# emmyoh/zebra

Hardware: AMD Instinct MI355X
Metric: queries/sec (higher is better)
Workload: dtype f32

## Files before the change

### zebra_amd/csrc/zh_api.hip

```cpp
#include <algorithm>
#include <atomic>
#include <chrono>
#include <condition_variable>
#include <cmath>
#include <deque>
#include <cstdarg>
#include <cstdio>
#include <cstring>
#include <mutex>
#include <shared_mutex>
#include <new>
#include <string>
#include <thread>
#include <vector>

#include "zh_internal.h"
#include "zh_snapfile.h"

static thread_local std::string g_err;

static int fail(int code, const char *fmt, ...) {
    char buf[512];
    va_list ap;
    va_start(ap, fmt);
    vsnprintf(buf, sizeof buf, fmt, ap);
    va_end(ap);
    g_err = buf;
    return code;
}
#define HIPCHK(expr)                                                                                       \
    do {                                                                                                   \
        hipError_t e_ = (expr);                                                                            \
        if (e_ != hipSuccess)                                                                              \
            return fail(e_ == hipErrorOutOfMemory ? ZH_ENOMEM : ZH_EHIP, "%s: %s (%s:%d)", #expr,          \
                        hipGetErrorString(e_), __FILE__, __LINE__);                                        \
    } while (0)

int zh_set_error(int code, const char *fmt, ...) {
    char buf[512];
    va_list ap;
    va_start(ap, fmt);
    vsnprintf(buf, sizeof buf, fmt, ap);
    va_end(ap);
    g_err = buf;
    return code;
}

extern "C" const char *zh_last_error(void) { return g_err.c_str(); }
extern "C" const char *zh_version(void) { return "zebra-hip 0.1 (gfx950)"; }

struct DevBuf {
    void *p = nullptr;
    size_t cap = 0;
    bool defer = false;
    std::vector<void *> old;
    size_t old_bytes = 0;
    int ensure(size_t bytes, bool keep = false, hipStream_t s = nullptr) {
        if (bytes <= cap) return ZH_OK;
        if (defer) bytes += bytes / 8;
        if (defer && old_bytes + cap > (size_t(2) << 30)) {
            for (void *o : old) hipFree(o);
            old.clear();
            old_bytes = 0;
        }
        size_t ncap = std::max(bytes, cap + cap / 2);
        ncap = (ncap + 255) & ~size_t(255);
        void *np = nullptr;
        hipError_t e = hipMalloc(&np, ncap);
        if (e != hipSuccess) {
            ncap = (bytes + 255) & ~size_t(255);
            e = hipMalloc(&np, ncap);
        }
        if (e != hipSuccess) return fail(ZH_ENOMEM, "hipMalloc(%zu bytes): %s", ncap, hipGetErrorString(e));
        if (keep && p && cap) {
            e = hipMemcpyAsync(np, p, cap, hipMemcpyDeviceToDevice, s);
            if (e == hipSuccess) e = hipStreamSynchronize(s);
            if (e != hipSuccess) { hipFree(np); return fail(ZH_EHIP, "grow copy: %s", hipGetErrorString(e)); }
        }
        if (p) { if (defer) { old.push_back(p); old_bytes += cap; } else hipFree(p); }
        p = np;
        cap = ncap;
        return ZH_OK;
    }
    void release() {
        if (p) hipFree(p);
        for (void *o : old) hipFree(o);
        old.clear();
        old_bytes = 0;
        p = nullptr;
        cap = 0;
    }
    template <typename T>
    T *as() const { return reinterpret_cast<T *>(p); }
};

struct zh_search_ctx {
    zh_index *ix = nullptr;
    DevBuf wQQ, wBits, wCounts, wInline, wRowBase, wCandBase, wVisitBase, wTotals, wVisits, wKeys, wCandKeys, wCandIds,
        wLeafCount, wLeafFill, wGroupBase, wGroupRowBase, wGroups, wGroupRowOff, wWaveGroup, wVisitBits, wNodeVisit, wScore, wJunkBits, wZeros, wQnorm, wQpad, wFixList, wLogPool, wLogHead, wLogCtl,
        wPfRows, wPfCounts, wPfKeys, wPfIds, wPfAmb, wPfCtl, wUnc, wQh, wQmeta, wApList, wApCount, wApEx, wApExKeys, wApCtl, wRaw;
    ZhApprox dbg_ap{};
    bool dbg_valid = false, dbg_raw = false;
    size_t log_chunks = 0;
    ZhTotals *h_totals = nullptr;
    hipEvent_t ev[6] = {};
    hipEvent_t ev_totals = nullptr, ev_emit = nullptr, ev_sw0 = nullptr, ev_sw1 = nullptr;
    bool ev_ok = false;
    int state = 0;
    bool trivial = false;
    const float *dQ = nullptr;
    size_t B = 0, k = 0;
    size_t nwin = 1, bwin = 0;
    DevBuf wQwin, wOutWin;
    int metric = 0, mode = 0;
    uint32_t P_dense = 0, wpq = 0;
    hipStream_t s = nullptr;
    ZhTotals tot{};
    bool scan = false;
    bool approx_f32rows = false;
    bool approx_fused = false;
    bool approx_bytes = false;
    bool approx = false, approx_mfma = false, approx_leaf = false;
    uint32_t *h_ap = nullptr;
    bool score_hash = false;
    uint32_t score_Bp = 0;
    bool lazy_fix = false;
    bool prefilter = false, prefilter_off_once = false, stream_ordered = false;
    uint32_t pf_cap = 0;
    uint32_t *h_pf = nullptr;
    std::vector<const float *> sv_q;
    std::vector<uint64_t *> sv_ids, sv_keys;
    std::vector<uint32_t *> sv_counts;
    hipStream_t sv_heavy = nullptr;
    std::vector<DevBuf *> all_bufs() {
        return {&wQQ, &wBits, &wCounts, &wInline, &wRowBase, &wCandBase, &wVisitBase, &wTotals, &wVisits, &wKeys,
                &wCandKeys, &wCandIds, &wLeafCount, &wLeafFill, &wGroupBase, &wGroupRowBase, &wGroups, &wGroupRowOff, &wWaveGroup, &wVisitBits, &wNodeVisit, &wScore, &wJunkBits, &wZeros, &wQnorm, &wQpad, &wFixList,
                &wLogPool, &wLogHead, &wLogCtl, &wQwin, &wOutWin, &wPfRows, &wPfCounts, &wPfKeys, &wPfIds, &wPfAmb, &wPfCtl, &wUnc,
                &wQh, &wQmeta, &wApList, &wApCount, &wApEx, &wApExKeys, &wApCtl, &wRaw};
    }
    void release_all() {
        for (DevBuf *b : all_bufs()) b->release();
        if (ev_ok) { for (auto &e : ev) hipEventDestroy(e); hipEventDestroy(ev_totals); hipEventDestroy(ev_emit); hipEventDestroy(ev_sw0); hipEventDestroy(ev_sw1); ev_ok = false; }
        if (h_totals) { hipHostFree(h_totals); h_totals = nullptr; }
        if (h_pf) { hipHostFree(h_pf); h_pf = nullptr; }
        if (h_ap) { hipHostFree(h_ap); h_ap = nullptr; }
    }
};

struct zh_index {
    zh_options opt{};
    int device = 0;
    hipStream_t stream = nullptr;
    hipStream_t sweep_stream = nullptr;
    std::shared_mutex mu;

    DevBuf X;
    uint64_t n_rows = 0;

    DevBuf node_plane, node_left, node_right, node_pack, roots, planes, consts, leaf_ids;
    uint32_t n_nodes = 0, n_planes = 0, n_trees = 0;
    uint64_t n_leaf_ids = 0;
    std::vector<int32_t> h_plane, h_left, h_right;
    std::vector<uint32_t> h_roots;
    std::vector<uint32_t> planes_below_level;
    std::vector<uint32_t> h_leaf_ids;
    std::vector<uint8_t> h_dead;
    uint64_t n_dead = 0;
    std::vector<uint32_t> h_live;
    uint64_t h_live_rows = ~0ull;
    uint64_t h_live_dead = ~0ull;
    uint64_t h_live_gen = ~0ull;
    uint64_t rows_gen = 1, dead_gen = 1;
    uint32_t max_leaf_len = 0;
    DevBuf blk_recs, blk_upper, blk_roots;
    uint32_t n_blocks = 0, n_upper = 0;
    bool blocks_valid = false;
    bool blocks_inner = false;
    size_t blk_recs_b = 0;
    std::mutex blk_mu;
    DevBuf row_leaf;
    bool row_leaf_valid = false, row_leaf_failed = false;
    std::atomic<uint32_t> batches_since_change{0};
    DevBuf row_half, row_meta, row_rho_dev;
    std::atomic<bool> row_half_failed{false};
    DevBuf row_half128;
    std::atomic<uint64_t> h128_rows{0}, h128_gen{0};
    int h128_ex = 0;
    float h128_rho = 0.f;
    std::atomic<bool> h128_failed{false};
    bool h128_bytes = false, h128_not_bytes = false;
    std::atomic<uint64_t> scale_rows{0}, scale_gen{0};
    float row_rho = 0.f;
    DevBuf scan_perm, row_leaf_p;
    bool row_order_off = false;
    uint32_t order_keys = 0;
    double order_worth = 0;
    uint64_t perm_rows = 0, row_leaf_gen = 0, row_leaf_p_gen = 0, perm_gen = 0, row_leaf_p_perm = 0;
    uint64_t row_leaf_rows = 0;

    zh_search_ctx dctx;
    DevBuf wQ, wOutIds, wOutKeys, wOutCounts;
    DevBuf ex_live, ex_bits, ex_QQ, ex_keys, ex_visits, ex_cbase, ex_ckeys, ex_cids, ex_run_ids, ex_run_keys, ex_run_counts, ex_Q, ex_ids, ex_kout, ex_counts,
        ex_Qh, ex_qmeta, ex_tau, ex_cnt, ex_lid, ex_llo, ex_lhi, ex_scr, ex_over;
    uint64_t ex_live_rows = ~0ull, ex_live_gen = ~0ull, ex_n_live = 0;
    zh_exact_info ex_info{};
    DevBuf fl_filter, fl_bits, fl_pos, fl_bcount, fl_bexcl, fl_tmp, fl_list;
    zh_filtered_info fl_info{};
    DevBuf rg_maxk, rg_cnt, rg_ctr, rg_pv0, rg_pv1, rg_pk0, rg_pk1, rg_cand, rg_tmp, rg_off, rg_oids, rg_okeys;
    zh_range_info rg_info{};
    DevBuf jn_ctr, jn_maxk, jn_tau, jn_pv0, jn_pv1, jn_pk0, jn_pk1, jn_qm, jn_cid, jn_first, jn_cand, jn_rows, jn_tmp, jn_oa, jn_ob, jn_okeys;
    zh_join_info jn_info{};
    DevBuf kn_qm, kn_cid, kn_pos, kn_A, kn_pmeta, kn_pid, kn_cbase, kn_pids, kn_pkeys, kn_pcounts, kn_oids, kn_okeys, kn_ocounts;
    zh_knn_info kn_info{};
    DevBuf fk_ntree, fk_rl, fk_flag, fk_excl, fk_tmp, fk_rows, fk_ctr, fk_lens, fk_takes, fk_rbase, fk_cbase, fk_groups, fk_groff, fk_segs, fk_colsrc, fk_crow,
        fk_hrow, fk_held, fk_CA, fk_cmeta, fk_cqm, fk_HA, fk_hmeta, fk_qrow, fk_maxk, fk_redo, fk_pos;
    zh_knn_forest_info fk_info{};
    DevBuf fj_leafof, fj_pieces, fj_linel, fj_linek, fj_segs, fj_cand;
    zh_join_forest_info fj_info{};

// ... 2082 lines not shown
    if (c->state != 1) return fail(ZH_ESTATE, "zh_search_finish without zh_search_begin");
    const uint32_t d = ix->opt.dim, T = ix->n_trees;
    const size_t B = c->B, k = c->k, nwin = c->nwin, bwin = c->bwin;
    hipStream_t s = c->s;
    int rc;
    c->state = 0;
    if (c->trivial) {
        for (size_t j = 0; j < nwin && bwin; j++) {
            HIPCHK(hipMemsetAsync(outCounts[j], 0, bwin * 4, s));
            if (k) {
                HIPCHK(hipMemsetAsync(outIds[j], 0xFF, bwin * k * 8, s));
                HIPCHK(hipMemsetAsync(outKeys[j], 0xFF, bwin * k * 8, s));
            }
        }
        HIPCHK(hipEventRecord(c->ev[5], s));
        c->state = 2;
        return ZH_OK;
    }
    uint64_t *dOutIds = outIds[0], *dOutKeys = outKeys[0];
    uint32_t *dOutCounts = outCounts[0];
    if (nwin > 1) {
        if ((rc = c->wOutWin.ensure(B * k * 16 + B * 4))) { return rc; }
        dOutIds = c->wOutWin.as<uint64_t>();
        dOutKeys = dOutIds + B * k;
        dOutCounts = reinterpret_cast<uint32_t *>(dOutKeys + B * k);
    }
    HIPCHK(hipEventSynchronize(c->ev_totals));
    const ZhTotals tot = c->tot = *c->h_totals;
    {
        std::lock_guard<std::mutex> lk(ix->stats_mu);
        const double v = (double)tot.visits / (double)((uint64_t)B * T);
        ix->visits_per_pair = ix->visits_per_pair > 0 ? 0.5 * (ix->visits_per_pair + v) : v;
    }
    if (tot.visits > 0xFFFFFFFull || tot.rows >= (1ull << 36))
        return fail(ZH_ELIMIT, "more than 2^28 leaf visits or 2^36 scored rows in one batch; use a smaller batch");
    c->sv_ids.assign(outIds, outIds + nwin); c->sv_keys.assign(outKeys, outKeys + nwin); c->sv_counts.assign(outCounts, outCounts + nwin);
    c->sv_heavy = heavy;
    if (c->prefilter && (tot.flags & 1u)) {
        const std::vector<const float *> q = c->sv_q;
        c->prefilter_off_once = true;
        rc = ctx_begin(c, q.data(), nwin, bwin, k, c->metric, c->mode, s);
        c->prefilter_off_once = false;
        if (rc) return rc;
        return ctx_finish(c, outIds, outKeys, outCounts, heavy);
    }
    if (c->prefilter) return finish_prefilter(c, dOutIds, dOutKeys, dOutCounts, outIds, outKeys, outCounts);
    if ((rc = c->wVisits.ensure(std::max<uint64_t>(tot.visits, 1) * sizeof(ZhVisit)))) return rc;
    if ((rc = c->wGroups.ensure(std::max<uint64_t>(tot.groups, 1) * sizeof(ZhGroup)))) return rc;
    if ((rc = c->wGroupRowOff.ensure(std::max<uint64_t>(tot.groups, 1) * 8))) return rc;
    if ((rc = c->wWaveGroup.ensure((tot.group_rows / 64 + 2) * 4))) return rc;
    if ((rc = c->wKeys.ensure(std::max<uint64_t>(tot.rows, 1) * 8))) return rc;
    if ((rc = c->wCandKeys.ensure(std::max<uint64_t>(tot.takes, 1) * 8))) return rc;
    if ((rc = c->wCandIds.ensure(std::max<uint64_t>(tot.takes, 1) * 4))) return rc;
    ZhForestDev f = forest_dev(ix);
    if (!(tot.flags & 1u)) {
        HIPCHK(zh_launch_expand(f, (uint32_t)B, c->wCounts.as<ZhPairCounts>(), c->wInline.as<ZhVisit>(),
                                c->wRowBase.as<uint64_t>(), c->wCandBase.as<uint64_t>(), c->wVisitBase.as<uint64_t>(),
                                c->wVisits.as<ZhVisit>(), c->wLeafCount.as<uint32_t>(), c->wLeafFill.as<uint32_t>(),
                                c->wGroupBase.as<uint32_t>(), c->wGroupRowBase.as<uint64_t>(), c->wGroups.as<ZhGroup>(),
                                c->wGroupRowOff.as<uint64_t>(), walk_log(c), s));
    } else {
        if (c->lazy_fix)
            HIPCHK(zh_launch_score_unc_fix(c->dQ, (uint32_t)B, d, f.planes, f.consts, ix->n_planes, c->wBits.as<uint32_t>(), c->wUnc.as<uint32_t>(), c->wpq, s));
        HIPCHK(zh_launch_walk_emit(f, c->dQ, (uint32_t)B, d, (int32_t)k, c->wBits.as<uint32_t>(), c->wpq, c->P_dense,
                                   c->wCounts.as<ZhPairCounts>(), c->wInline.as<ZhVisit>(), c->wRowBase.as<uint64_t>(),
                                   c->wCandBase.as<uint64_t>(), c->wVisitBase.as<uint64_t>(), c->wVisits.as<ZhVisit>(),
                                   c->wLeafCount.as<uint32_t>(), c->wLeafFill.as<uint32_t>(), c->wGroupBase.as<uint32_t>(),
                                   c->wGroupRowBase.as<uint64_t>(), c->wGroups.as<ZhGroup>(), c->wGroupRowOff.as<uint64_t>(), s));
        const uint64_t pairs = (uint64_t)B * T;
        const uint64_t want = tot.visits / (ZH_LOG_CHUNK - 1) + std::min<uint64_t>(pairs, tot.visits / (ZH_INLINE_VISITS + 1)) + 16;
        static const bool fixed = getenv("ZH_WALK_LOG_FIXED") != nullptr;
        if (!fixed && want > c->log_chunks) {
            const size_t chunks = (size_t)(want + want / 2);
            if (c->wLogPool.ensure(chunks * ZH_LOG_CHUNK * sizeof(uint2)) == ZH_OK) c->log_chunks = chunks;
        }
    }
    c->scan = choose_scan(ix, tot, c->metric, B, k);
    if (c->scan && (!ix->row_leaf_valid || ix->row_leaf_rows != ix->n_rows)) {
        std::lock_guard<std::mutex> lk(ix->blk_mu);
        if ((!ix->row_leaf_valid || ix->row_leaf_rows != ix->n_rows) && !ix->row_leaf_failed && (rc = build_row_leaf(ix))) return rc;
        if (!ix->row_leaf_valid || ix->row_leaf_rows != ix->n_rows) c->scan = false;
    }
    if (c->scan) {
        const size_t nn = std::max<uint32_t>(ix->n_nodes, 1);
        if ((rc = c->wVisitBits.ensure((nn + 31) / 32 * 4))) return rc;
        if ((rc = c->wNodeVisit.ensure(nn * sizeof(uint4)))) return rc;
        HIPCHK(zh_launch_node_visits(c->wLeafCount.as<uint32_t>(), c->wGroupBase.as<uint32_t>(), c->wGroups.as<ZhGroup>(), ix->n_nodes,
                                     c->wVisitBits.as<uint32_t>(), c->wNodeVisit.as<uint4>(), s));
    }
    if (!c->scan)
        HIPCHK(zh_launch_wave_groups(c->wGroups.as<ZhGroup>(), c->wGroupRowOff.as<uint64_t>(), tot.groups, c->wWaveGroup.as<uint32_t>(), s));
    c->approx = c->scan && use_approx(ix, tot, B, k, c->metric);
    c->approx_leaf = false; c->approx_bytes = false;
    if (!c->scan && use_approx_leaf(ix, tot, B, k, c->metric)) {
        bool ok = false;
        const char *be = getenv("ZH_S128H_BYTES"), *ke = getenv("ZH_S128H_KERNEL"), *de = getenv("ZH_S128H_DMA");
        const bool want_bytes = !(be && be[0] == '0') && !(ke && ke[0] == 'r') && !(de && de[0] == '1');
        std::lock_guard<std::mutex> lk(ix->blk_mu);
        if ((rc = ensure_row_half128(ix, &ok, want_bytes))) return rc;
        c->approx = c->approx_leaf = ok;
        c->approx_bytes = ok && ix->h128_bytes;
    }
    ZhApprox ap{};
    bool mfma = c->approx && !c->approx_leaf && mfma_wanted(ix) && B < (1u << 23) - 1;
    const uint2 *scan_row_leaf = ix->row_leaf.as<uint2>();
    if (mfma) {
        std::lock_guard<std::mutex> lk(ix->blk_mu);
        if ((rc = ensure_row_half(ix, &mfma))) return rc;
        if (mfma && ix->perm_rows) {
            if ((rc = ensure_row_leaf_p(ix))) return rc;
            if (!ix->perm_rows) {
                ix->row_order_off = true;
                ix->scale_gen = 0;
                if ((rc = ensure_row_half(ix, &mfma))) return rc;
            } else
                scan_row_leaf = ix->row_leaf_p.as<uint2>();
        }
    }
    c->approx_mfma = mfma;
    c->approx_f32rows = mfma && ix->row_half.p == nullptr;
    if (c->approx) {
        const char *cap_e = getenv("ZH_APX_CAPS");
        unsigned e_capq = 0, e_excap = 0, e_exrows = 0;
        if (cap_e) sscanf(cap_e, "%u,%u,%u", &e_capq, &e_excap, &e_exrows);
        const uint32_t capq = e_capq ? std::min(e_capq, 8192u) : (ix->approx_strikes.load() ? 8192u : 4096u);
        const uint32_t ex_cap = e_excap ? e_excap : (uint32_t)std::min<uint64_t>(std::max<uint64_t>(4096, tot.visits / 4 + 1024), 1u << 24);
        const uint32_t ex_rows = e_exrows ? e_exrows : (uint32_t)std::min<uint64_t>(std::max<uint64_t>(1u << 20, tot.rows / 16), 1u << 26);
        if ((rc = c->wQh.ensure(B * d * 2)) || (rc = c->wQmeta.ensure(B * sizeof(float4))) || (rc = c->wApList.ensure((size_t)B * capq * 12)) ||
            (rc = c->wApCount.ensure(B * 8 + std::max<uint64_t>(tot.visits, 1) * 4)) || (rc = c->wApEx.ensure((size_t)ex_cap * 8)) || (rc = c->wApExKeys.ensure((size_t)ex_rows * 20)) ||
            (rc = c->wApCtl.ensure(ZH_APX_CTL_WORDS * 4)))
            return rc;
        ap.Qh = c->wQh.p; ap.qmeta = c->wQmeta.as<float4>(); ap.iv = c->wKeys.as<uint64_t>();
        ap.list_lo = c->wApList.as<uint32_t>(); ap.list_hi = ap.list_lo + (size_t)B * capq; ap.list_id = ap.list_hi + (size_t)B * capq;
        ap.qcount = c->wApCount.as<uint32_t>(); ap.capq = capq; ap.qtau = ap.qcount + B; ap.tauv = ap.qtau + B;
        ap.ex_visits = c->wApEx.as<uint2>(); ap.ex_cap = ex_cap;
        ap.ex_keys = c->wApExKeys.as<uint64_t>(); ap.ex_ckeys = ap.ex_keys + ex_rows; ap.ex_cids = reinterpret_cast<uint32_t *>(ap.ex_ckeys + ex_rows);
        ap.ex_rows_cap = ex_rows; ap.ctl = c->wApCtl.as<uint32_t>();
        ap.n_queries = (uint32_t)B; ap.iv_cap = tot.rows;
        ap.mfma = mfma ? 1u : 0u; ap.row_half = mfma ? ix->row_half.p : nullptr; ap.row_meta = mfma ? ix->row_meta.as<float2>() : nullptr;
        ap.row_rho = mfma ? ix->row_rho : 0.f;
        if (c->approx_leaf) { ap.mfma = 2u; ap.row_rho = ap.rho_norm = c->approx_bytes ? 0.f : ix->h128_rho; }
        const char *pte = getenv("ZH_S128H_PRETEST");
        ap.nx_max = c->approx_leaf && c->approx_bytes && !(pte && pte[0] == '0') ? 2885.1f : 0.f;
        HIPCHK(hipMemsetAsync(c->wApCount.p, 0, B * 4, s));
        HIPCHK(hipMemsetAsync(ap.qtau, 0xFF, B * 4, s));
        HIPCHK(hipMemsetAsync(c->wApCtl.p, 0, ZH_APX_CTL_WORDS * 4, s));
        HIPCHK(zh_launch_qhalf(c->dQ, (uint32_t)B, d, c->wQh.p, c->wQmeta.as<float4>(), c->approx_leaf ? 2 : (mfma ? 1 : 0), s));
    }
    HIPCHK(hipEventRecord(c->ev[2], s));
    hipStream_t hs = heavy ? heavy : s;
    if (hs != s) { HIPCHK(hipEventRecord(c->ev_emit, s)); HIPCHK(hipStreamWaitEvent(hs, c->ev_emit, 0)); }
    HIPCHK(hipEventRecord(c->ev_sw0, hs));
    c->approx_fused = false;
    if (c->approx_leaf && k <= 64 && !ix->debug_keep_raw) {
        const char *fe = getenv("ZH_S128H_FUSED"), *ke = getenv("ZH_S128H_KERNEL"), *de = getenv("ZH_S128H_DMA");
        const bool lean = !(ke && ke[0] == 'r') && !(de && de[0] == '1');
        c->approx_fused = lean && (fe ? fe[0] == '1' : (!ix->fused_off && tot.rows >= 1024 * std::max<uint64_t>(tot.visits, 1)));
    }
    const int kinda = c->metric != ZH_COSINE ? 0 : (c->mode == ZH_COSINE_PARITY ? 2 : 1);
    if (c->approx_leaf)
        HIPCHK(zh_launch_sweep128h(ix->row_half128.p, c->wQh.p, ldexpf(1.f, ix->h128_ex - 14), c->wGroups.as<ZhGroup>(), c->wGroupRowOff.as<uint64_t>(),
                                   tot.groups, c->wWaveGroup.as<uint32_t>(), f.leaf_ids, tot.group_rows, c->wKeys.as<uint64_t>(), hs,
                                   c->approx_fused ? &ap : nullptr, kinda, (uint32_t)k, zh_approx_bound(c->metric, d, 2), c->approx_bytes));
    else if (c->approx)
        HIPCHK(zh_launch_scan_approx(ix->X.as<float>(), d, ix->n_rows, ap, mfma ? scan_row_leaf : ix->row_leaf.as<uint2>(), T, c->wVisitBits.as<uint32_t>(),
                                     c->wNodeVisit.as<uint4>(), c->wGroups.as<ZhGroup>(), f.group, c->metric, c->mode, hs));
    else if (c->scan)
        HIPCHK(zh_launch_scan_sweep(ix->X.as<float>(), d, ix->n_rows, c->dQ, c->wQQ.as<float>(), ix->row_leaf.as<uint2>(), T,
                                    c->wVisitBits.as<uint32_t>(), c->wNodeVisit.as<uint4>(), c->wGroups.as<ZhGroup>(), f.group,
                                    c->metric, c->mode, c->wKeys.as<uint64_t>(), nullptr, hs));
    else
        HIPCHK(zh_launch_sweep(ix->X.as<float>(), d, c->dQ, c->wQQ.as<float>(), c->wGroups.as<ZhGroup>(),
                               c->wGroupRowOff.as<uint64_t>(), tot.groups, c->wWaveGroup.as<uint32_t>(), f.leaf_ids,
                               tot.group_rows, c->metric, c->mode, c->wKeys.as<uint64_t>(), hs));
    HIPCHK(hipEventRecord(c->ev_sw1, hs));
    if (hs != s) HIPCHK(hipStreamWaitEvent(s, c->ev_sw1, 0));
    HIPCHK(hipEventRecord(c->ev[3], s));
    const uint32_t *run_if = nullptr;
    c->dbg_valid = c->approx;
    c->dbg_raw = false;
    if (c->approx) {
        c->dbg_ap = ap;
        if (ix->debug_keep_raw && tot.rows) {
            if ((rc = c->wRaw.ensure(tot.rows * 8))) return rc;
            HIPCHK(hipMemcpyAsync(c->wRaw.p, c->wKeys.p, tot.rows * 8, hipMemcpyDeviceToDevice, s));
            c->dbg_raw = true;
        }
        if (c->approx_fused) HIPCHK(zh_launch_exact_register(c->wVisits.as<ZhVisit>(), tot.visits, (uint32_t)k, ap, s));
        else HIPCHK(zh_launch_select_interval(c->wVisits.as<ZhVisit>(), tot.visits, (uint32_t)k, f.leaf_ids, ap, c->metric, c->mode, d, s));
        HIPCHK(hipEventRecord(c->ev[4], s));
        HIPCHK(zh_launch_final_interval(c->wVisits.as<ZhVisit>(), ix->X.as<float>(), d, c->dQ, c->wQQ.as<float>(), (uint32_t)B, (uint32_t)k,
                                        f.leaf_ids, c->metric, c->mode, ix->opt.id_base, ap, dOutIds, dOutKeys, dOutCounts, ix->max_leaf_len, s));
        HIPCHK(hipMemcpyAsync(c->h_ap, c->wApCtl.p, ZH_APX_CTL_WORDS * 4, hipMemcpyDeviceToHost, s));
        run_if = ap.ctl + 1;
        if (c->approx_leaf)
            HIPCHK(zh_launch_sweep(ix->X.as<float>(), d, c->dQ, c->wQQ.as<float>(), c->wGroups.as<ZhGroup>(), c->wGroupRowOff.as<uint64_t>(), tot.groups,
                                   c->wWaveGroup.as<uint32_t>(), f.leaf_ids, tot.group_rows, c->metric, c->mode, c->wKeys.as<uint64_t>(), s, run_if));
        else
            HIPCHK(zh_launch_scan_sweep(ix->X.as<float>(), d, ix->n_rows, c->dQ, c->wQQ.as<float>(), ix->row_leaf.as<uint2>(), T,
                                        c->wVisitBits.as<uint32_t>(), c->wNodeVisit.as<uint4>(), c->wGroups.as<ZhGroup>(), f.group,
                                        c->metric, c->mode, c->wKeys.as<uint64_t>(), run_if, s));
    }
    HIPCHK(zh_launch_select(c->wVisits.as<ZhVisit>(), tot.visits, f.leaf_ids, c->wKeys.as<uint64_t>(),
                            c->wCandKeys.as<uint64_t>(), c->wCandIds.as<uint32_t>(), ix->max_leaf_len, run_if, s));
    if (!c->approx) HIPCHK(hipEventRecord(c->ev[4], s));
    HIPCHK(zh_launch_final(c->wCandBase.as<uint64_t>(), (uint32_t)B, T, (uint32_t)k, c->wCandKeys.as<uint64_t>(),
                           c->wCandIds.as<uint32_t>(), ix->opt.id_base, dOutIds, dOutKeys, dOutCounts, run_if, s));
    for (size_t j = 0; j < nwin && nwin > 1; j++) {
        HIPCHK(hipMemcpyAsync(outIds[j], dOutIds + j * bwin * k, bwin * k * 8, hipMemcpyDeviceToDevice, s));
        HIPCHK(hipMemcpyAsync(outKeys[j], dOutKeys + j * bwin * k, bwin * k * 8, hipMemcpyDeviceToDevice, s));
        HIPCHK(hipMemcpyAsync(outCounts[j], dOutCounts + j * bwin, bwin * 4, hipMemcpyDeviceToDevice, s));
    }
    HIPCHK(hipEventRecord(c->ev[5], s));
    c->state = 2;
    return ZH_OK;
}

int ctx_wait(zh_search_ctx *c) {
    zh_index *ix = c->ix;
    if (c->state == 1) return fail(ZH_ESTATE, "zh_search_wait: the batch was begun but not finished");
    if (c->state != 2) return ZH_OK;
    c->state = 0;
    HIPCHK(hipEventSynchronize(c->ev[5]));
    if (c->trivial) return ZH_OK;
    const bool pf = c->prefilter;
    const uint32_t pf_amb = pf ? c->h_pf[0] : 0, pf_flags = pf ? c->h_pf[1] : 0, pf_exact = pf ? c->h_pf[2] : 0;
    if (pf_flags) {
        {
            std::lock_guard<std::mutex> lk(ix->stats_mu);
            ix->stats.prefilter_fallbacks_accum++;
            ix->stats.prefilter_last_overflow = pf_flags;
        }
        ix->prefilter_strikes.fetch_add(1);
        const std::vector<const float *> q = c->sv_q;
        const std::vector<uint64_t *> ids = c->sv_ids, keys = c->sv_keys;
        const std::vector<uint32_t *> counts = c->sv_counts;
        c->prefilter_off_once = true;
        int rc = ctx_begin(c, q.data(), c->nwin, c->bwin, c->k, c->metric, c->mode, c->s);
        if (!rc) rc = ctx_finish(c, ids.data(), keys.data(), counts.data(), c->sv_heavy);
        c->prefilter_off_once = false;
        if (rc) return rc;
        return ctx_wait(c);
    }
    if (pf) ix->prefilter_strikes = 0;
    const ZhTotals tot = c->tot;
    uint64_t uniq = 0;
    if (ix->profiling >= 2 && tot.visits && !pf) {
        std::vector<ZhVisit> hv(tot.visits);
        HIPCHK(hipMemcpy(hv.data(), c->wVisits.p, tot.visits * sizeof(ZhVisit), hipMemcpyDeviceToHost));
        std::vector<std::pair<uint32_t, uint32_t>> leaves(hv.size());
        for (size_t i = 0; i < hv.size(); i++) leaves[i] = {hv[i].leaf_off, hv[i].len};
        std::sort(leaves.begin(), leaves.end());
        leaves.erase(std::unique(leaves.begin(), leaves.end()), leaves.end());
        for (auto &l : leaves) uniq += l.second;
    }
    float ms[5] = {0, 0, 0, 0, 0};
    if (ix->profiling > 0) {
        for (int i = 0; i < 5; i++) HIPCHK(hipEventElapsedTime(&ms[i], c->ev[i], c->ev[i + 1]));
        HIPCHK(hipEventElapsedTime(&ms[2], c->ev_sw0, c->ev_sw1));
    }
    std::lock_guard<std::mutex> lk(ix->stats_mu);
    zh_stats_t &st = ix->stats;
    st.batch = c->B; st.window_batches = c->nwin; st.visits = tot.visits; st.rows_scored = tot.rows; st.candidates = tot.takes;
    st.planes_dense = c->P_dense; st.planes_total = ix->n_planes;
    const uint64_t swept = pf ? pf_exact : (c->scan ? ix->n_rows : tot.group_rows);
    st.rows_swept = swept;
    st.sweep_bytes = pf ? tot.rows * 64 + (uint64_t)pf_exact * 4 * ix->opt.dim
                        : (c->scan ? ix->n_rows * ((uint64_t)4 * ix->opt.dim + 8 * ix->n_trees) + tot.rows * 8
                                   : tot.group_rows * ((uint64_t)4 * ix->opt.dim + 4) + tot.rows * 8);
    st.table_scan = c->scan && !pf ? 1 : 0;
    const bool apx = c->approx && !pf;
    st.approx_scan = apx ? (c->approx_leaf ? 3 : (c->approx_mfma ? 2 : 1)) : 0;
    st.approx_fused = apx && c->approx_leaf && c->approx_fused ? 1 : 0;
    st.approx_byte_rows = apx && c->approx_leaf && c->approx_bytes ? 1 : 0;
    st.approx_exact_visits = apx ? c->h_ap[0] : 0;
    st.approx_survivors = apx ? c->h_ap[3] : 0;
    st.approx_list_entries = apx ? c->h_ap[4] : 0;
    if (apx && c->h_ap[7]) fprintf(stderr, "zebra_hip: scan guard tripped, bits %u (diagnostic build)\n", c->h_ap[7]);
    st.approx_columns = apx && c->approx_mfma ? c->h_ap[5] : 0;
    st.approx_column_pairs = apx && c->approx_mfma ? c->h_ap[6] : 0;
    if (apx && c->h_ap[1]) {
        st.approx_fallbacks_accum++;
        st.approx_last_overflow = c->h_ap[1];
// ... 2303 lines not shown
```

### zebra_amd/csrc/zh_approx.hip

```cpp

#include <cstdlib>

#include "zh_internal.h"
#include "zh_device.h"

typedef _Float16 f16x8 __attribute__((ext_vector_type(8)));

#ifndef ZH_APX_G768
#define ZH_APX_G768 2
#endif
#ifndef ZH_APX_G128
#define ZH_APX_G128 8
#endif
uint32_t zh_approx_groups(uint32_t d) {
    switch (d) {
    case 128: return ZH_APX_G128;
    case 256: case 384: return 4;
    case 768: return ZH_APX_G768;
    case 512: case 1024: return 2;
    default: return 0;
    }
}
bool zh_approx_pays(uint32_t d) { return d >= 384; }

float zh_approx_bound(int metric, uint32_t d, int mfma) {
    const double u = 5.9604644775390625e-8, c0 = (d + 255) / 256 + 8.0, ops = mfma ? 33.0 * (d / 128) + 2.0 + (mfma == 2 ? 40.0 : 0.0) : 0.0;
    if (metric == ZH_COSINE) return (float)(1.01 * (2.0 * c0 + 80.0 + 2.0 * ops) * u);
    return (float)(1.01 * (c0 + 100.0 + ops) * u);
}

__device__ __forceinline__ _Float16 f16_no_subnormal(float v) {
    const _Float16 h = (_Float16)v;
    return fabsf((float)h) < 6.103515625e-05f ? (_Float16)0.f : h;
}

template <int G>
__global__ __launch_bounds__(64) void qhalf_kernel(const float *__restrict__ Q, uint32_t B, uint32_t d, _Float16 *__restrict__ Qh,
                                                    float4 *__restrict__ qmeta) {
    constexpr uint32_t LG = 64 / G;
    const uint32_t b = blockIdx.x, lane = threadIdx.x;
    const float *q = Q + (size_t)b * d;
    float m = 0.f, s2 = 0.f;
    bool bad = false;
    for (uint32_t e = lane; e < d; e += 64) {
        const float v = q[e];
        bad |= !(v - v == 0.f);
        m = fmaxf(m, fabsf(v));
        s2 = __builtin_fmaf(v, v, s2);
    }
    m = wave_butterfly<OpMax>(m);
    s2 = wave_sum_canonical(s2);
    bad = __ballot(bad) != 0;
    float sigma = 1.f, inv = 1.f;
    if (!bad && m > 0.f) {
        int ex = 0;
        (void)frexpf(m, &ex);
        if (ex < -90 || ex > 90) bad = true;
        else { sigma = ldexpf(1.f, 14 - ex); inv = ldexpf(1.f, ex - 14); }
    }
    float d2 = 0.f;
    for (uint32_t e = lane; e < d; e += 64) {
        const float v = bad ? 0.f : q[e];
        const _Float16 h = f16_no_subnormal(v * sigma);
        const float df = v - (float)h * inv;
        d2 = __builtin_fmaf(df, df, d2);
        const uint32_t j = e / (4 * LG), rem = e % (4 * LG), l = rem / 4, t = rem % 4, i = j / 2, wh = j % 2;
        Qh[(size_t)b * d + ((size_t)(i * LG + l)) * 8 + wh * 4 + t] = h;
    }
    d2 = wave_sum_canonical(d2);
    if (lane == 0) {
        float4 o;
        if (bad || !(s2 - s2 == 0.f)) o = make_float4(NAN, NAN, NAN, NAN);
        else o = make_float4(inv, s2, sqrtf(s2) * (1.0f + 1e-5f), sqrtf(d2) * 1.001f);
        qmeta[b] = o;
    }
}

hipError_t zh_launch_qhalf(const float *dQ, uint32_t B, uint32_t d, void *dQh, float4 *dQmeta, int layout, hipStream_t s) {
    if (!B) return hipSuccess;
    const uint32_t G = layout == 2 ? 64 : (layout == 1 ? 16 : zh_approx_groups(d));
    if (G == 64) hipLaunchKernelGGL(qhalf_kernel<64>, dim3(B), dim3(64), 0, s, dQ, B, d, (_Float16 *)dQh, dQmeta);
    else if (G == 16) hipLaunchKernelGGL(qhalf_kernel<16>, dim3(B), dim3(64), 0, s, dQ, B, d, (_Float16 *)dQh, dQmeta);
    else if (G == 8) hipLaunchKernelGGL(qhalf_kernel<8>, dim3(B), dim3(64), 0, s, dQ, B, d, (_Float16 *)dQh, dQmeta);
    else if (G == 4) hipLaunchKernelGGL(qhalf_kernel<4>, dim3(B), dim3(64), 0, s, dQ, B, d, (_Float16 *)dQh, dQmeta);
    else if (G == 2) hipLaunchKernelGGL(qhalf_kernel<2>, dim3(B), dim3(64), 0, s, dQ, B, d, (_Float16 *)dQh, dQmeta);
    else return hipErrorInvalidValue;
    return hipGetLastError();
}

template <int LG>
__device__ __forceinline__ float group_sum(float s) {
    s = s + dpp_mov<0xB1>(s);
    s = s + dpp_mov<0x4E>(s);
    s = s + dpp_mov<0x141>(s);
    if (LG >= 16) s = s + dpp_mov<0x140>(s);
    if (LG >= 32) s = xor16<OpAdd>(s);
    if (LG >= 64) {
        const auto r = __builtin_amdgcn_permlane32_swap(__float_as_uint(s), __float_as_uint(s), false, false);
        s = __uint_as_float(r[0]) + __uint_as_float(r[1]);
    }
    return s;
}


__device__ __forceinline__ uint32_t scan_phase1(uint32_t lane, uint32_t n_ent, const uint2 *__restrict__ ent,
                                                const uint32_t *__restrict__ visitBits, const uint4 *__restrict__ nodeVisit,
                                                uint32_t *eGb, uint32_t *eWithin, uint32_t *eC, uint32_t *off, uint32_t *eB0, uint64_t *eK0) {
    unsigned long long rlw[ZH_SCAN_NE];
#pragma unroll
    for (int j = 0; j < ZH_SCAN_NE; j++) {
        const uint32_t e = lane + 64u * j;
        rlw[j] = __builtin_nontemporal_load(reinterpret_cast<const unsigned long long *>(ent + (e < n_ent ? e : 0)));
    }
    uint32_t word[ZH_SCAN_NE];
    bool in[ZH_SCAN_NE];
#pragma unroll
    for (int j = 0; j < ZH_SCAN_NE; j++) {
        const uint32_t node = (uint32_t)rlw[j];
        in[j] = lane + 64u * j < n_ent && node != 0xFFFFFFFFu;
        word[j] = visitBits[in[j] ? node >> 5 : 0];
    }
    uint4 nv[ZH_SCAN_NE];
#pragma unroll
    for (int j = 0; j < ZH_SCAN_NE; j++) {
        const uint32_t node = (uint32_t)rlw[j];
        in[j] = in[j] && ((word[j] >> (node & 31)) & 1u);
        nv[j] = nodeVisit[in[j] ? node : 0];
    }
    uint32_t P = 0;
#pragma unroll
    for (int j = 0; j < ZH_SCAN_NE; j++) {
        eWithin[j] = (uint32_t)(rlw[j] >> 32);
        eC[j] = in[j] ? nv[j].x & 0x0FFFFFFFu : 0u;
        eGb[j] = nv[j].y; eB0[j] = nv[j].z;
        eK0[j] = ((uint64_t)(nv[j].x >> 28) << 32) | nv[j].w;
        uint32_t incl = eC[j];
#pragma unroll
        for (int o = 1; o < 64; o <<= 1) {
            const uint32_t t = __shfl_up(incl, o);
            if (lane >= (uint32_t)o) incl += t;
        }
        off[j] = P + incl - eC[j];
        P += (uint32_t)__builtin_amdgcn_readlane((int)incl, 63);
    }
    return P;
}

#define ZH_APX_CAP 512
#ifndef ZH_APX_WAVES
#define ZH_APX_WAVES 0
#endif
#ifndef ZH_APX_REPL_ROWS
#define ZH_APX_REPL_ROWS 0
#endif
template <int D, int G, int KINDA>
__global__ __launch_bounds__(256)
#if ZH_APX_WAVES
__attribute__((amdgpu_waves_per_eu(ZH_APX_WAVES, 8)))
#endif
void scan_approx_kernel(const float *__restrict__ X, const uint4 *__restrict__ Qh,
                                                           const float4 *__restrict__ qmeta, const uint2 *__restrict__ rowLeaf,
                                                           uint32_t T, uint32_t RW, const uint32_t *__restrict__ visitBits,
                                                           const uint4 *__restrict__ nodeVisit, const ZhGroup *__restrict__ groups,
                                                           uint32_t GRP, uint64_t row_begin, uint64_t row_end, float Kc,
                                                           uint64_t *__restrict__ iv) {
    constexpr int LG = 64 / G, NH = D * G / 512, NR = 2 * NH;
    constexpr int RB = NR <= 6 ? 4 : 2;
    static_assert(D * G % 512 == 0 && NH >= 1, "a lane's share of a query is whole 16-byte loads");
    __shared__ uint4 pair_list[4][ZH_APX_CAP];
    __shared__ uint32_t row_start[4][20];
    const uint32_t lane = threadIdx.x & 63, l = lane & (LG - 1), g = lane / LG;
    const uint32_t wid = (uint32_t)__builtin_amdgcn_readfirstlane((int)(threadIdx.x >> 6));
    const uint64_t wave = (uint64_t)blockIdx.x * (blockDim.x >> 6) + wid;
    const uint64_t r0 = row_begin + wave * RW;
    if (r0 >= row_end) return;
    const uint32_t nr = (uint32_t)(row_end - r0 < RW ? row_end - r0 : RW);
    const uint32_t n_ent = nr * T;
    const uint2 *__restrict__ ent = rowLeaf + (size_t)r0 * T;
    uint32_t eGb[ZH_SCAN_NE], eWithin[ZH_SCAN_NE], eC[ZH_SCAN_NE], off[ZH_SCAN_NE], eB0[ZH_SCAN_NE];
    uint64_t eK0[ZH_SCAN_NE];
    const uint32_t P = scan_phase1(lane, n_ent, ent, visitBits, nodeVisit, eGb, eWithin, eC, off, eB0, eK0);
    if (P == 0) return;
    const float4 *__restrict__ X4 = reinterpret_cast<const float4 *>(X);
    float my_s = 0.f, my_a2 = 0.f;
    uint64_t my_slot = 0;
    uint32_t nst = 0;
    bool my_on = false;
    auto flush = [&]() {
        if (my_on) __builtin_nontemporal_store(((uint64_t)__float_as_uint(my_a2) << 32) | __float_as_uint(my_s), iv + my_slot);
        my_on = false;
        nst = 0;
    };
    auto load_q = [&](uint32_t b, uint4 *hq) {
        const uint4 *qp = Qh + (size_t)b * (D / 8) + l;
#pragma unroll
        for (int i = 0; i < NH; i++) hq[i] = qp[i * LG];
    };
    auto load_x = [&](uint64_t row, float4 *v) {
        if constexpr (G == 2 && !ZH_APX_REPL_ROWS) {
            const float4 *r4 = X4 + (size_t)row * (D / 4) + lane;
#pragma unroll
            for (int j = 0; j < NR / 2; j++) {
                const float4 t = ld16<true>(r4 + 64 * j);
                const auto sx = __builtin_amdgcn_permlane32_swap(__float_as_uint(t.x), __float_as_uint(t.x), false, false);
                const auto sy = __builtin_amdgcn_permlane32_swap(__float_as_uint(t.y), __float_as_uint(t.y), false, false);
                const auto sz = __builtin_amdgcn_permlane32_swap(__float_as_uint(t.z), __float_as_uint(t.z), false, false);
                const auto sw = __builtin_amdgcn_permlane32_swap(__float_as_uint(t.w), __float_as_uint(t.w), false, false);
                v[2 * j] = make_float4(__uint_as_float(sx[0]), __uint_as_float(sy[0]), __uint_as_float(sz[0]), __uint_as_float(sw[0]));
                v[2 * j + 1] = make_float4(__uint_as_float(sx[1]), __uint_as_float(sy[1]), __uint_as_float(sz[1]), __uint_as_float(sw[1]));
            }
        } else {
            const float4 *r4 = X4 + (size_t)row * (D / 4) + l;
#pragma unroll
            for (int j = 0; j < NR; j++) v[j] = ld16<true>(r4 + LG * j);
        }
    };
    auto row_sumsq = [&](const float4 *v) {
        float4 c = make_float4(0.f, 0.f, 0.f, 0.f);
#pragma unroll
        for (int j = 0; j < NR; j++) sq4(v[j], c);
        return group_sum<LG>((c.x + c.y) + (c.z + c.w));
    };
    auto dot_h = [&](const float4 *v, const uint4 *hq) {
        float ax = 0.f, ay = 0.f, az = 0.f, aw = 0.f;
#pragma unroll
        for (int i = 0; i < NH; i++) {
            f16x8 h;
            __builtin_memcpy(&h, &hq[i], 16);
            ax = __builtin_fmaf(v[2 * i].x, (float)h[0], ax);
            ay = __builtin_fmaf(v[2 * i].y, (float)h[1], ay);
            az = __builtin_fmaf(v[2 * i].z, (float)h[2], az);
            aw = __builtin_fmaf(v[2 * i].w, (float)h[3], aw);
            ax = __builtin_fmaf(v[2 * i + 1].x, (float)h[4], ax);
            ay = __builtin_fmaf(v[2 * i + 1].y, (float)h[5], ay);
            az = __builtin_fmaf(v[2 * i + 1].z, (float)h[6], az);
            aw = __builtin_fmaf(v[2 * i + 1].w, (float)h[7], aw);
        }
        return group_sum<LG>((ax + ay) + (az + aw));
    };
    auto stash = [&](float s, float a2, uint32_t, uint64_t slot, bool valid) {
        if (l == nst) { my_s = s; my_a2 = a2; my_slot = slot; my_on = valid; }
        if (++nst == (uint32_t)LG) flush();
    };
    if (P <= ZH_APX_CAP) {
        uint4 *list = pair_list[wid];
        uint32_t *rstart = row_start[wid];
        uint32_t mrows = 0;
#pragma unroll
        for (int j = 0; j < ZH_SCAN_NE; j++) {
            const uint32_t e = lane + 64u * j, c = eC[j];
            if (e < n_ent && e % T == 0) rstart[e / T] = off[j];
            if (c) {
                const uint32_t rl = e / T, gb = eGb[j];
                mrows |= 1u << rl;
                {
                    const uint64_t slot = eK0[j] + eWithin[j];
                    list[off[j]] = make_uint4(rl, eB0[j], (uint32_t)slot, (uint32_t)(slot >> 32));
                }
                for (uint32_t sidx = 1; sidx < c; sidx++) {
                    const ZhGroup *gp = groups + gb + sidx / GRP;
                    const uint64_t slot = gp->key_off[sidx % GRP] + eWithin[j];
                    list[off[j] + sidx] = make_uint4(rl, gp->b[sidx % GRP], (uint32_t)slot, (uint32_t)(slot >> 32));
                }
            }
// ... 95 lines not shown
        for (uint32_t e = lane; e < d; e += 64) {
            const float v = x[e];
            bad |= !(v - v == 0.f);
            m = fmaxf(m, fabsf(v));
            a2 = __builtin_fmaf(v, v, a2);
        }
        m = wave_butterfly<OpMax>(m);
        a2 = wave_sum_canonical(a2);
        bad = __ballot(bad) != 0;
        bool usable = false;
        float sigma = 1.f, inv = __uint_as_float(0x7FC00000u);
        if (!bad) {
            int ex = 14;
            if (m > 0.f) (void)frexpf(m, &ex);
            if (ex >= -100 && ex <= 100) { usable = true; sigma = ldexpf(1.f, 14 - ex); inv = ldexpf(1.f, ex - 14); }
        }
        float s2 = 0.f, d2 = 0.f;
        _Float16 *tile = Xh + ((size_t)(row >> 4) * NS * 64 + (row & 15)) * 8;
        for (uint32_t e = lane; e < d; e += 64) {
            const float v = x[e] * sigma;
            const _Float16 hv = usable ? f16_no_subnormal(v) : (_Float16)0.f;
            const float df = v - (float)hv;
            s2 = __builtin_fmaf(v, v, s2);
            d2 = __builtin_fmaf(df, df, d2);
            const uint32_t st = e >> 5, w = e & 31, hh = (w & 15) >> 2, j = (w & 3) + ((w >> 4) << 2);
            if (Xh) tile[((size_t)st * 64 + hh * 16) * 8 + j] = hv;
        }
        s2 = wave_sum_canonical(s2);
        d2 = wave_sum_canonical(d2);
        if (usable && s2 > 0.f) rho_w = fmaxf(rho_w, sqrtf(d2) * 1.001f / (sqrtf(s2) * 0.9999f));
        if (lane == 0) rowMeta[row] = make_float2(a2, inv);
    }
    if (lane == 0 && rho_w > 0.f) atomicMax(rhoMax, __float_as_uint(rho_w));
}

hipError_t zh_launch_row_half(const float *dX, uint64_t row0, uint64_t n_rows, uint32_t d, void *dXh, float2 *dRowMeta, uint32_t *dRhoMax,
                              const uint32_t *dPerm, uint64_t perm_rows, hipStream_t s) {
    if (!n_rows) return hipSuccess;
    const uint64_t blocks = std::min<uint64_t>((n_rows + 3) / 4, 256 * 32);
    hipLaunchKernelGGL(row_half_kernel, dim3((uint32_t)blocks), dim3(256), 0, s, dX, row0, n_rows, d, (_Float16 *)dXh, dRowMeta, dRhoMax, dPerm, perm_rows);
    return hipGetLastError();
}

__global__ __launch_bounds__(256) void permute_row_leaf_kernel(const uint2 *__restrict__ rowLeaf, const uint32_t *__restrict__ perm, uint64_t perm_rows,
                                                               uint64_t n_entries, uint32_t T, uint2 *__restrict__ out) {
    for (uint64_t e = (uint64_t)blockIdx.x * blockDim.x + threadIdx.x; e < n_entries; e += (uint64_t)gridDim.x * blockDim.x) {
        const uint64_t p = e / T, t = e % T;
        out[e] = rowLeaf[(size_t)(p < perm_rows ? perm[p] : p) * T + t];
    }
}
hipError_t zh_launch_permute_row_leaf(const uint2 *dRowLeaf, const uint32_t *dPerm, uint64_t perm_rows, uint64_t n_rows, uint32_t T, uint2 *dOut, hipStream_t s) {
    const uint64_t n = n_rows * T;
    if (!n) return hipSuccess;
    hipLaunchKernelGGL(permute_row_leaf_kernel, dim3((uint32_t)std::min<uint64_t>((n + 255) / 256, 256 * 64)), dim3(256), 0, s, dRowLeaf, dPerm, perm_rows, n, T, dOut);
    return hipGetLastError();
}

#ifndef ZH_MFMA_CL
#define ZH_MFMA_CL 0
#endif
#ifdef ZH_SCAN_GUARD
#define ZH_GUARD(cond, bit) ((cond) ? true : (atomicOr(guard, (bit)), false))
#else
#define ZH_GUARD(cond, bit) true
#endif
#ifdef ZH_SCAN_PROF
__device__ unsigned long long zh_scan_prof_buf[16];
extern "C" __attribute__((visibility("default"))) int zh_debug_scan_prof(uint64_t *out, uint32_t words, int reset) {
    static const unsigned long long zero[16] = {};
    if (reset) return (int)hipMemcpyToSymbol(HIP_SYMBOL(zh_scan_prof_buf), zero, sizeof(zero));
    return (int)hipMemcpyFromSymbol(out, HIP_SYMBOL(zh_scan_prof_buf), (size_t)words * 8);
}
#define SP(...) __VA_ARGS__
#else
#define SP(...)
#endif
#ifndef ZH_MFMA_WAVES
#define ZH_MFMA_WAVES 3
#endif
template <int D, bool F32ROWS>
__global__ __launch_bounds__(256) __attribute__((amdgpu_waves_per_eu(D > 768 ? 2 : ZH_MFMA_WAVES, D > 768 ? 2 : ZH_MFMA_WAVES)))
void scan_mfma_kernel(const u32x4v *__restrict__ Xh, const float *__restrict__ Xf, const float2 *__restrict__ rowMeta,
                                                         const uint4 *__restrict__ Qh, const uint2 *__restrict__ rowLeaf, uint32_t T,
                                                         uint32_t RW, const uint32_t *__restrict__ visitBits,
                                                         const uint4 *__restrict__ nodeVisit, const ZhGroup *__restrict__ groups,
                                                         uint32_t GRP, uint64_t row_begin, uint64_t row_end, uint64_t *__restrict__ iv,
                                                         uint32_t *__restrict__ colStats ,
                                                         uint32_t nq, uint64_t iv_cap, uint32_t *__restrict__ guard) {
    constexpr int NS = D / 32;
    constexpr int NL = D / 64;
    constexpr int CL = ZH_MFMA_CL ? ZH_MFMA_CL : (NL % 4 == 0 ? 2 : 3);
    constexpr int NCH = NL / CL;
    static_assert(D % 128 == 0 && NL % CL == 0 && NCH % 2 == 0, "four accumulators; the chunk registers alternate with a static parity");
    __shared__ uint64_t pair_list[4][ZH_APX_CAP > CL * 256 ? ZH_APX_CAP : CL * 256];
    __shared__ uint64_t tile_list[4][ZH_APX_CAP];
    __shared__ uint32_t col_query[4][ZH_APX_CAP];
    __shared__ uint32_t tile_start[4][36];
    __shared__ f32x4v acc_lds[4][64];
    __shared__ float2 row_meta[4][16];
    const uint32_t lane = threadIdx.x & 63, c16 = lane & 15, h = lane >> 4;
    const uint32_t wid = (uint32_t)__builtin_amdgcn_readfirstlane((int)(threadIdx.x >> 6));
    const uint64_t wave = (uint64_t)blockIdx.x * (blockDim.x >> 6) + wid;
    const uint64_t r0 = row_begin + wave * RW;
    if (r0 >= row_end) return;
    SP(const uint64_t sp0 = clock64();)
    const uint32_t nr = (uint32_t)(row_end - r0 < RW ? row_end - r0 : RW);
    const uint32_t n_ent = nr * T;
    const uint2 *__restrict__ ent = rowLeaf + (size_t)r0 * T;
    uint32_t eGb[ZH_SCAN_NE], eWithin[ZH_SCAN_NE], eC[ZH_SCAN_NE], off[ZH_SCAN_NE], eB0[ZH_SCAN_NE];
    uint64_t eK0[ZH_SCAN_NE];
    const uint32_t P = scan_phase1(lane, n_ent, ent, visitBits, nodeVisit, eGb, eWithin, eC, off, eB0, eK0);
    if (P == 0) return;
    SP(const uint64_t sp1 = clock64();)
    uint64_t *list = pair_list[wid];
    const bool listed = P <= ZH_APX_CAP;
    auto pack = [](uint32_t rl, uint32_t b, uint64_t slot) { return slot | ((uint64_t)b << 36) | ((uint64_t)rl << 60); };
#pragma unroll
    for (int j = 0; j < ZH_SCAN_NE; j++) {
        const uint32_t e = lane + 64u * j, c = eC[j];
        if (c && listed && ZH_GUARD(off[j] + c <= (uint32_t)ZH_APX_CAP && e / T < 16u, 32u)) {
            const uint32_t rl = e / T, gb = eGb[j];
            list[off[j]] = pack(rl, eB0[j], eK0[j] + eWithin[j]);
            for (uint32_t sidx = 1; sidx < c; sidx++) {
                const ZhGroup *gp = groups + gb + sidx / GRP;
                list[off[j] + sidx] = pack(rl, gp->b[sidx % GRP], gp->key_off[sidx % GRP] + eWithin[j]);
            }
        }
    }
    SP(__builtin_amdgcn_s_waitcnt(0); const uint64_t sp2 = clock64();)
    f16x8 A[NS];
    if constexpr (!F32ROWS) {
        const u32x4v *tp = Xh + (size_t)(r0 >> 4) * (NS * 64) + lane;
#pragma unroll
        for (int st = 0; st < NS; st++) A[st] = __builtin_bit_cast(f16x8, __builtin_nontemporal_load(tp + 64 * st));
        if (lane < 16) row_meta[wid][lane] = rowMeta[r0 + (lane < nr ? lane : 0u)];
        __builtin_amdgcn_fence(__ATOMIC_RELEASE, "wavefront");
        __builtin_amdgcn_wave_barrier();
    } else {
        if (lane < 16) row_meta[wid][lane] = rowMeta[r0 + (lane < nr ? lane : 0u)];
        __builtin_amdgcn_fence(__ATOMIC_RELEASE, "wavefront");
        __builtin_amdgcn_wave_barrier();
        const float inv_c = row_meta[wid][c16].y;
        const bool usable_c = inv_c - inv_c == 0.f;
        const float sigma_c = usable_c ? 1.0f / inv_c : 0.f;
        f32x4v *xt = reinterpret_cast<f32x4v *>(tile_list[wid]);
        const f32x4v *X4 = reinterpret_cast<const f32x4v *>(Xf);
        const uint32_t g4 = lane >> 4, p16 = lane & 15;
        auto cvt8 = [&](const f32x4v lo, const f32x4v hi) {
            f16x8 o;
#pragma unroll
            for (int t = 0; t < 4; t++) {
                o[t] = usable_c ? f16_no_subnormal(lo[t] * sigma_c) : (_Float16)0.f;
                o[4 + t] = usable_c ? f16_no_subnormal(hi[t] * sigma_c) : (_Float16)0.f;
            }
            return o;
        };
        f32x4v Rr[4];
        auto issue_rows = [&](int kb) {
#pragma unroll
            for (int i = 0; i < 4; i++) {
                const uint32_t rr = 4u * i + g4;
                Rr[i] = __builtin_nontemporal_load(X4 + (size_t)(r0 + (rr < nr ? rr : nr - 1)) * (D / 4) + kb * 16 + p16);
            }
        };
        issue_rows(0);
#pragma unroll
        for (int kb = 0; kb < D / 64; kb++) {
#pragma unroll
            for (int i = 0; i < 4; i++) {
                const uint32_t rr = 4u * i + g4;
                xt[rr * 16 + (p16 ^ rr)] = Rr[i];
            }
            __builtin_amdgcn_fence(__ATOMIC_RELEASE, "wavefront");
            __builtin_amdgcn_wave_barrier();
            if (kb + 1 < D / 64) issue_rows(kb + 1);
#pragma unroll
            for (int s2 = 0; s2 < 2; s2++) {
                const f32x4v lo = xt[c16 * 16 + ((8u * s2 + h) ^ c16)], hi = xt[c16 * 16 + ((8u * s2 + 4u + h) ^ c16)];
                A[2 * kb + s2] = cvt8(lo, hi);
            }
            __builtin_amdgcn_fence(__ATOMIC_RELEASE, "wavefront");
            __builtin_amdgcn_wave_barrier();
        }
    }
    const float2 *rmeta = row_meta[wid];
    u32x4v *stg = reinterpret_cast<u32x4v *>(pair_list[wid]);
    const u32x4v *__restrict__ Qv = reinterpret_cast<const u32x4v *>(Qh);
    const uint32_t g8 = lane >> 3, pc = lane & 7;
    const uint32_t swA = (g8 >> 1) & 7u, swB = (4u + (g8 >> 1)) & 7u;
    const uint32_t rd0 = (c16 >> 3) * 64u + (c16 & 7u) * 8u + ((h ^ (c16 >> 1)) & 7u);
    const uint32_t rd1 = (c16 >> 3) * 64u + (c16 & 7u) * 8u + (((4u + h) ^ (c16 >> 1)) & 7u);
    auto issue = [&](uint32_t bA, uint32_t bB, int chunk, u32x4v *dst) {
        if (!ZH_GUARD(bA < nq && bB < nq, 1u)) { bA = 0; bB = 0; }
        const u32x4v *qa = Qv + (size_t)bA * (D / 8) + (size_t)(chunk * CL * 8) + (pc ^ swA);
// ... 101 lines not shown
        }
        __builtin_amdgcn_fence(__ATOMIC_RELEASE, "wavefront");
        __builtin_amdgcn_wave_barrier();
        const uint32_t nt = (nd + 15) / 16;
        SP(const uint64_t sp3 = clock64();)
        if (colStats && lane == 0 && (wave & 63u) == 0u) { atomicAdd(&colStats[0], nd); atomicAdd(&colStats[1], P); }
        auto col_b = [&](uint32_t t, uint32_t col) { const uint32_t ci = 16 * t + col; return colq[ci < nd ? ci : nd - 1]; };
        uint32_t bA = col_b(0, g8), bB = col_b(0, 8 + g8);
        u32x4v ra[2 * CL], rb[2 * CL];
        issue(bA, bB, 0, ra);
        SP(__builtin_amdgcn_s_waitcnt(0); const uint64_t sp4 = clock64();)
        f32x4v *al = acc_lds[wid];
        for (uint32_t t = 0; t < nt; t++) {
            f32x4v acc[4] = {{0.f, 0.f, 0.f, 0.f}, {0.f, 0.f, 0.f, 0.f}, {0.f, 0.f, 0.f, 0.f}, {0.f, 0.f, 0.f, 0.f}};
#pragma unroll
            for (int c = 0; c < NCH; c += 2) {
                issue(bA, bB, c + 1, rb);
                to_lds(ra);
                mfma_chunk(c, acc);
                if (c + 2 < NCH) issue(bA, bB, c + 2, ra);
                else {
                    bA = col_b(t + 1, g8); bB = col_b(t + 1, 8 + g8);
                    issue(bA, bB, 0, ra);
                }
                to_lds(rb);
                mfma_chunk(c + 1, acc);
            }
            al[c16 * 4 + h] = (acc[0] + acc[1]) + (acc[2] + acc[3]);
            __builtin_amdgcn_fence(__ATOMIC_RELEASE, "wavefront");
            __builtin_amdgcn_wave_barrier();
            const uint32_t pe = tstart[t + 1];
            for (uint32_t pi = tstart[t] + lane; pi < pe; pi += 64) {
                const uint64_t rec = tl[pi];
                const uint32_t rl = (uint32_t)(rec >> 60), col = (uint32_t)(rec >> 36) & 15u;
                const float sv = reinterpret_cast<const float *>(al)[col * 16 + rl];
                const float2 rm = rmeta[rl];
                if (ZH_GUARD((rec & 0xFFFFFFFFFull) < iv_cap, 2u))
                    __builtin_nontemporal_store(((uint64_t)__float_as_uint(rm.x) << 32) | __float_as_uint(sv * rm.y), iv + (rec & 0xFFFFFFFFFull));
            }
            __builtin_amdgcn_wave_barrier();
        }
        SP(if ((wave & 15u) == 0u && lane == 0) {
            __builtin_amdgcn_s_waitcnt(0);
            const uint64_t sp5 = clock64();
            atomicAdd(&zh_scan_prof_buf[0], 1ull); atomicAdd(&zh_scan_prof_buf[1], sp1 - sp0); atomicAdd(&zh_scan_prof_buf[2], sp2 - sp1);
            atomicAdd(&zh_scan_prof_buf[3], sp3 - sp2); atomicAdd(&zh_scan_prof_buf[4], sp4 - sp3); atomicAdd(&zh_scan_prof_buf[5], sp5 - sp4);
            atomicAdd(&zh_scan_prof_buf[6], (unsigned long long)nt); atomicAdd(&zh_scan_prof_buf[7], (unsigned long long)P);
            atomicAdd(&zh_scan_prof_buf[8], (unsigned long long)nd); atomicAdd(&zh_scan_prof_buf[9], sp5 - sp0);
        })
    } else {
#pragma unroll
        for (int j = 0; j < ZH_SCAN_NE; j++) {
            unsigned long long m = __ballot(eC[j] != 0);
            while (m) {
                const int ll = __builtin_ctzll(m);
                m &= m - 1;
                const uint32_t c = (uint32_t)__builtin_amdgcn_readlane((int)eC[j], ll);
                const uint32_t gb = (uint32_t)__builtin_amdgcn_readlane((int)eGb[j], ll);
                const uint32_t w = (uint32_t)__builtin_amdgcn_readlane((int)eWithin[j], ll);
                const uint32_t rl = ((uint32_t)ll + 64u * j) / T;
                for (uint32_t s0 = 0; s0 < c; s0 += 16) {
                    auto visit_b = [&](uint32_t col) { const uint32_t si = s0 + col < c ? s0 + col : c - 1; return groups[gb + si / GRP].b[si % GRP]; };
                    const uint32_t bA = visit_b(g8), bB = visit_b(8 + g8);
                    const uint32_t sidx = s0 + c16 < c ? s0 + c16 : c - 1;
                    const ZhGroup *gp = groups + gb + sidx / GRP;
                    f32x4v acc[4] = {{0.f, 0.f, 0.f, 0.f}, {0.f, 0.f, 0.f, 0.f}, {0.f, 0.f, 0.f, 0.f}, {0.f, 0.f, 0.f, 0.f}};
                    u32x4v rq[2 * CL];
#pragma unroll
                    for (int cc = 0; cc < NCH; cc++) {
                        issue(bA, bB, cc, rq);
                        to_lds(rq);
                        mfma_chunk(cc, acc);
                        __builtin_amdgcn_sched_barrier(0);
                    }
                    emit(acc, rl, gp->key_off[sidx % GRP] + w, s0 + c16 < c);
                }
            }
        }
    }
}

template <int D>
static hipError_t launch_scan_mfma_d(const float *dX, uint64_t n_rows, const ZhApprox &ap, const uint2 *dRowLeaf, uint32_t T,
                                     const uint32_t *dVisitBits, const uint4 *dNodeVisit, const ZhGroup *dGroups, uint32_t group, hipStream_t s) {
    const uint32_t RW = zh_scan_rows_per_wave(T);
    uint64_t rows_per_launch = zh_sweep_rows_per_launch(D);
    rows_per_launch = rows_per_launch / (4 * RW) * (4 * RW);
    for (uint64_t r = 0; r < n_rows; r += rows_per_launch) {
        const uint64_t r_end = r + rows_per_launch < n_rows ? r + rows_per_launch : n_rows;
        const uint64_t waves = (r_end - r + RW - 1) / RW, blocks = (waves + 3) / 4;
        if (blocks > 0x7FFFFFFFull) return hipErrorInvalidValue;
        if (ap.row_half)
            hipLaunchKernelGGL((scan_mfma_kernel<D, false>), dim3((uint32_t)blocks), dim3(256), 0, s, (const u32x4v *)ap.row_half, dX, ap.row_meta, (const uint4 *)ap.Qh, dRowLeaf, T, RW,
                               dVisitBits, dNodeVisit, dGroups, group, r, r_end, ap.iv, ap.ctl + 5, ap.n_queries, ap.iv_cap, ap.ctl + 7);
        else
            hipLaunchKernelGGL((scan_mfma_kernel<D, true>), dim3((uint32_t)blocks), dim3(256), 0, s, (const u32x4v *)nullptr, dX, ap.row_meta, (const uint4 *)ap.Qh, dRowLeaf, T, RW,
                               dVisitBits, dNodeVisit, dGroups, group, r, r_end, ap.iv, ap.ctl + 5, ap.n_queries, ap.iv_cap, ap.ctl + 7);
    }
    return hipGetLastError();
}

__global__ __launch_bounds__(256) void absmax_kernel(const float *__restrict__ X, uint64_t n, uint32_t *__restrict__ out) {
    float m = 0.f;
    for (uint64_t i = (uint64_t)blockIdx.x * blockDim.x + threadIdx.x; i < n; i += (uint64_t)gridDim.x * blockDim.x) {
        const float v = fabsf(X[i]);
        if (v - v == 0.f) m = fmaxf(m, v);
    }
    m = wave_butterfly<OpMax>(m);
    if ((threadIdx.x & 63) == 0 && m > 0.f) atomicMax(out, __float_as_uint(m));
}

__global__ __launch_bounds__(256) void row_half128_kernel(const float *__restrict__ X, uint64_t row0, uint64_t n_rows, float sigma,
                                                          _Float16 *__restrict__ Xh, uint32_t *__restrict__ rhoMax) {
    const uint32_t lane = threadIdx.x & 63;
    const uint64_t nw = (uint64_t)gridDim.x * 4;
    float rho_w = 0.f;
    for (uint64_t i = (uint64_t)blockIdx.x * 4 + (threadIdx.x >> 6); i < n_rows; i += nw) {
        const uint64_t row = row0 + i;
        const float2 x = reinterpret_cast<const float2 *>(X + (size_t)row * 128)[lane];
        const float v0 = x.x * sigma, v1 = x.y * sigma;
        bool bad = !(v0 - v0 == 0.f) || !(v1 - v1 == 0.f) || fabsf(v0) > 60000.f || fabsf(v1) > 60000.f;
        const _Float16 h0 = f16_no_subnormal(v0), h1 = f16_no_subnormal(v1);
        const float d0 = v0 - (float)h0, d1 = v1 - (float)h1;
        const float s2 = wave_sum_canonical(__builtin_fmaf(v0, v0, v1 * v1));
        const float d2 = wave_sum_canonical(__builtin_fmaf(d0, d0, d1 * d1));
        const float m = wave_butterfly<OpMax>(fmaxf(fabsf(x.x), fabsf(x.y)));
        bad = __ballot(bad) != 0 || !(s2 - s2 == 0.f) || (s2 == 0.f && m > 0.f);
        const float rho = s2 > 0.f ? sqrtf(d2) * 1.001f / (sqrtf(s2) * 0.9999f) : 0.f;
        bad = bad || !(rho <= 9.765625e-4f);
        if (!bad) rho_w = fmaxf(rho_w, rho);
        const _Float16 nanh = (_Float16)__uint_as_float(0x7FC00000u);
        typedef _Float16 f16x2v __attribute__((ext_vector_type(2)));
        reinterpret_cast<f16x2v *>(Xh + (size_t)row * 128)[lane] = bad ? f16x2v{nanh, nanh} : f16x2v{h0, h1};
    }
    if (lane == 0 && rho_w > 0.f) atomicMax(rhoMax, __float_as_uint(rho_w));
}

hipError_t zh_launch_absmax(const float *dX, uint64_t n, uint32_t *dOut, hipStream_t s) {
    if (!n) return hipSuccess;
    hipLaunchKernelGGL(absmax_kernel, dim3((uint32_t)std::min<uint64_t>((n + 255) / 256, 256 * 16)), dim3(256), 0, s, dX, n, dOut);
    return hipGetLastError();
}
hipError_t zh_launch_row_half128(const float *dX, uint64_t row0, uint64_t n_rows, float sigma, void *dXh, uint32_t *dRhoMax, hipStream_t s) {
    if (!n_rows) return hipSuccess;
    hipLaunchKernelGGL(row_half128_kernel, dim3((uint32_t)std::min<uint64_t>((n_rows + 3) / 4, 256 * 32)), dim3(256), 0, s, dX, row0, n_rows, sigma,
                       (_Float16 *)dXh, dRhoMax);
    return hipGetLastError();
}

__global__ __launch_bounds__(256) void row_byte128_kernel(const float4 *__restrict__ X4, uint64_t n4, uint32_t *__restrict__ Xb,
                                                          uint32_t *__restrict__ notBytes) {
    bool bad = false;
    for (uint64_t i = (uint64_t)blockIdx.x * 256 + threadIdx.x; i < n4; i += (uint64_t)gridDim.x * 256) {
        const float4 v = X4[i];
        const float e[4] = {v.x, v.y, v.z, v.w};
        uint32_t w = 0;
#pragma unroll
        for (int j = 0; j < 4; j++) {
            const uint32_t b = (uint32_t)fminf(fmaxf(e[j], 0.f), 255.f);
            bad |= !((float)b == e[j]);
            w |= b << (8 * j);
        }
        Xb[i] = w;
    }
    if (__ballot(bad) != 0 && (threadIdx.x & 63) == 0) atomicOr(notBytes, 1u);
}
hipError_t zh_launch_row_byte128(const float *dX, uint64_t row0, uint64_t n_rows, void *dXb, uint32_t *dNotBytes, hipStream_t s) {
    if (!n_rows) return hipSuccess;
    const uint64_t n4 = n_rows * 32;
    hipLaunchKernelGGL(row_byte128_kernel, dim3((uint32_t)std::min<uint64_t>((n4 + 255) / 256, 256 * 32)), dim3(256), 0, s,
                       reinterpret_cast<const float4 *>(dX + (size_t)row0 * 128), n4, reinterpret_cast<uint32_t *>(dXb) + (size_t)row0 * 32, dNotBytes);
    return hipGetLastError();
}
__device__ __forceinline__ f16x8 bytes8_to_f16(uint32_t w0, uint32_t w1) {
    typedef _Float16 h2 __attribute__((ext_vector_type(2)));
    const h2 off = {(_Float16)-1024.f, (_Float16)-1024.f};
    const h2 a = __builtin_bit_cast(h2, __builtin_amdgcn_perm(0x64646464u, w0, 0x04010400u)) + off;
    const h2 b = __builtin_bit_cast(h2, __builtin_amdgcn_perm(0x64646464u, w0, 0x04030402u)) + off;
    const h2 c = __builtin_bit_cast(h2, __builtin_amdgcn_perm(0x64646464u, w1, 0x04010400u)) + off;
    const h2 d = __builtin_bit_cast(h2, __builtin_amdgcn_perm(0x64646464u, w1, 0x04030402u)) + off;
// ... 880 lines not shown
#define ZH_S128L_CH 4
#endif
#ifndef ZH_S128F_CH
#define ZH_S128F_CH 16
#endif
#ifndef ZH_S128H_LAUNCH_X
#define ZH_S128H_LAUNCH_X 4
#endif
#ifndef ZH_S128B_LAUNCH_X
#define ZH_S128B_LAUNCH_X 8
#endif
#ifndef ZH_S128B_CH
#define ZH_S128B_CH 64
#endif
uint64_t zh_sweep128h_rows_per_launch(bool lean, bool byte_rows) {
    return (lean ? (byte_rows ? ZH_S128B_LAUNCH_X : ZH_S128H_LAUNCH_X) : 1) * zh_sweep_rows_per_launch(128);
}
template <int FUSE, bool BYTES>
static void launch_sweep128h_lean(const void *dXh, const void *dQh, float inv, const ZhGroup *dGroups, const uint64_t *dGroupRowOff, uint64_t n_groups,
                                  const uint32_t *dWaveGroup, const uint32_t *dLeafIds, uint64_t R_grouped, uint64_t *dIv, const ZhApprox &ap,
                                  uint32_t k_top, float Kc, hipStream_t s) {
    const uint64_t rows_per_launch = zh_sweep128h_rows_per_launch(true, BYTES);
    for (uint64_t r = 0; r < R_grouped; r += rows_per_launch) {
        const uint64_t r_end = r + rows_per_launch < R_grouped ? r + rows_per_launch : R_grouped;
        constexpr int CHL = FUSE >= 0 ? (BYTES ? ZH_S128B_CH : ZH_S128F_CH) : ZH_S128L_CH;
        const uint64_t wl = (r_end - r + 64 * CHL - 1) / (64 * CHL);
        if constexpr (BYTES)
            hipLaunchKernelGGL((sweep128b_lean_kernel<CHL, FUSE>), dim3((uint32_t)((wl + 3) / 4)), dim3(256), 0, s, (const u32x4v *)dXh,
                               (const u32x4v *)dQh, dGroups, dGroupRowOff, n_groups, dWaveGroup, dLeafIds, r, r_end, dIv, ap, k_top, Kc);
        else
            hipLaunchKernelGGL((sweep128h_lean_kernel<CHL, FUSE>), dim3((uint32_t)((wl + 3) / 4)), dim3(256), 0, s, (const u32x4v *)dXh,
                               (const u32x4v *)dQh, inv, dGroups, dGroupRowOff, n_groups, dWaveGroup, dLeafIds, r, r_end, dIv, ap, k_top, Kc);
    }
    const uint64_t bw = ((R_grouped + 63) / 64 + 63) / 64, bb = (bw + 3) / 4;
    hipLaunchKernelGGL((sweep128h_boundary_kernel<FUSE, BYTES>), dim3((uint32_t)bb), dim3(256), 0, s, (const u32x4v *)dXh, (const u32x4v *)dQh, inv, dGroups,
                       dGroupRowOff, n_groups, dWaveGroup, dLeafIds, (uint64_t)0, R_grouped, dIv, ap, k_top, Kc);
}
hipError_t zh_launch_sweep128h(const void *dXh, const void *dQh, float inv, const ZhGroup *dGroups, const uint64_t *dGroupRowOff, uint64_t n_groups,
                               const uint32_t *dWaveGroup, const uint32_t *dLeafIds, uint64_t R_grouped, uint64_t *dIv, hipStream_t s,
                               const ZhApprox *fuse, int fuse_kinda, uint32_t k_top, float Kc, bool byte_rows) {
    if (R_grouped == 0 || n_groups == 0) return hipSuccess;
    constexpr int CH = 4;
    const uint64_t rows_per_launch = zh_sweep_rows_per_launch(128);
    if ((R_grouped + 16383) / 16384 > 0x7FFFFFFFull) return hipErrorInvalidValue;
    const char *dma_e = getenv("ZH_S128H_DMA"), *kern_e = getenv("ZH_S128H_KERNEL");
    const bool dma = dma_e && dma_e[0] == '1', r5 = kern_e && kern_e[0] == 'r';
    if (fuse) {
        if (!dWaveGroup || k_top == 0 || k_top > 64) return hipErrorInvalidValue;
#define ZH_LEAN(F)                                                                                                                                  \
    do {                                                                                                                                            \
        if (byte_rows) launch_sweep128h_lean<F, true>(dXh, dQh, 1.f, dGroups, dGroupRowOff, n_groups, dWaveGroup, dLeafIds, R_grouped, dIv, *fuse, k_top, Kc, s); \
        else launch_sweep128h_lean<F, false>(dXh, dQh, inv, dGroups, dGroupRowOff, n_groups, dWaveGroup, dLeafIds, R_grouped, dIv, *fuse, k_top, Kc, s);           \
    } while (0)
        if (fuse_kinda == 0) ZH_LEAN(0);
        else if (fuse_kinda == 1) ZH_LEAN(1);
        else ZH_LEAN(2);
#undef ZH_LEAN
        return hipGetLastError();
    }
    if (!dma && !r5) {
        const ZhApprox none{};
        if (byte_rows) launch_sweep128h_lean<-1, true>(dXh, dQh, 1.f, dGroups, dGroupRowOff, n_groups, dWaveGroup, dLeafIds, R_grouped, dIv, none, 0u, 0.f, s);
        else launch_sweep128h_lean<-1, false>(dXh, dQh, inv, dGroups, dGroupRowOff, n_groups, dWaveGroup, dLeafIds, R_grouped, dIv, none, 0u, 0.f, s);
        return hipGetLastError();
    }
    if (byte_rows) return hipErrorInvalidValue;
    for (uint64_t r = 0; r < R_grouped; r += rows_per_launch) {
        const uint64_t r_end = r + rows_per_launch < R_grouped ? r + rows_per_launch : R_grouped;
        const uint64_t w = (r_end - r + 64 * CH - 1) / (64 * CH), blocks = (w + 3) / 4;
        if (!dma)
            hipLaunchKernelGGL((sweep128h_kernel<CH>), dim3((uint32_t)blocks), dim3(256), 0, s, (const u32x4v *)dXh, (const u32x4v *)dQh, inv, dGroups,
                               dGroupRowOff, n_groups, dWaveGroup, dLeafIds, r, r_end, dIv);
        else
            hipLaunchKernelGGL((sweep128h_dma_kernel<CH>), dim3((uint32_t)blocks), dim3(256), 0, s, (const u32x4v *)dXh, (const u32x4v *)dQh, inv, dGroups,
                               dGroupRowOff, n_groups, dWaveGroup, dLeafIds, r, r_end, dIv);
    }
    return hipGetLastError();
}


template <int G, int KINDA>
__global__ __launch_bounds__(256) void scan_approx128_kernel(const float *__restrict__ X, const uint4 *__restrict__ Qh,
                                                              const float4 *__restrict__ qmeta, const uint2 *__restrict__ rowLeaf,
                                                              uint32_t T, uint32_t RW, const uint32_t *__restrict__ visitBits,
                                                              const uint4 *__restrict__ nodeVisit, const ZhGroup *__restrict__ groups,
                                                              uint32_t GRP, uint64_t row_begin, uint64_t row_end, float Kc,
                                                              uint64_t *__restrict__ iv) {
    constexpr int LG = 64 / G, NH = G / 4, NR = 2 * NH;
    constexpr uint32_t CAP = 240;
    __shared__ uint64_t pair_list[4][CAP];
    __shared__ float4 row_lds[4][16 * 32];
    __shared__ float a2_lds[4][16];
    const uint32_t lane = threadIdx.x & 63, l = lane & (LG - 1), g = lane / LG;
    const uint32_t wid = (uint32_t)__builtin_amdgcn_readfirstlane((int)(threadIdx.x >> 6));
    const uint64_t wave = (uint64_t)blockIdx.x * (blockDim.x >> 6) + wid;
    const uint64_t r0 = row_begin + wave * RW;
    if (r0 >= row_end) return;
    const uint32_t nr = (uint32_t)(row_end - r0 < RW ? row_end - r0 : RW);
    const uint32_t n_ent = nr * T;
    const uint2 *__restrict__ ent = rowLeaf + (size_t)r0 * T;
    uint32_t eGb[ZH_SCAN_NE], eWithin[ZH_SCAN_NE], eC[ZH_SCAN_NE], off[ZH_SCAN_NE], eB0[ZH_SCAN_NE];
    uint64_t eK0[ZH_SCAN_NE];
    const uint32_t P = scan_phase1(lane, n_ent, ent, visitBits, nodeVisit, eGb, eWithin, eC, off, eB0, eK0);
    if (P == 0) return;
    {
        const float4 *src = reinterpret_cast<const float4 *>(X) + (size_t)r0 * 32;
        float4 t[8];
#pragma unroll
        for (int i = 0; i < 8; i++) t[i] = (lane + 64u * i < nr * 32u) ? ld16<true>(src + lane + 64 * i) : make_float4(0.f, 0.f, 0.f, 0.f);
#pragma unroll
        for (int i = 0; i < 8; i++) row_lds[wid][lane + 64 * i] = t[i];
    }
    __builtin_amdgcn_fence(__ATOMIC_RELEASE, "wavefront");
    __builtin_amdgcn_wave_barrier();
#pragma unroll
    for (int rr = 0; rr < 16 / G; rr++) {
        const uint32_t row = g + (uint32_t)G * rr;
        float4 c = make_float4(0.f, 0.f, 0.f, 0.f);
#pragma unroll
        for (int j = 0; j < NR; j++) sq4(row_lds[wid][row * 32 + LG * j + l], c);
        const float a2 = group_sum<LG>((c.x + c.y) + (c.z + c.w));
        if (l == 0) a2_lds[wid][row] = a2;
    }
    float my_s = 0.f;
    uint64_t my_slot = 0;
    uint32_t my_row = 0, nst = 0;
    bool my_on = false;
    auto flush = [&]() {
        if (my_on) __builtin_nontemporal_store(((uint64_t)__float_as_uint(a2_lds[wid][my_row]) << 32) | __float_as_uint(my_s), iv + my_slot);
        my_on = false;
        nst = 0;
    };
    struct Ops { float4 v[NR]; uint4 hq[NH]; };
    auto fetch = [&](uint32_t row, uint32_t b, Ops &o) {
#pragma unroll
        for (int i = 0; i < NH; i++) o.hq[i] = Qh[(size_t)b * 16 + i * LG + l];
#pragma unroll
        for (int j = 0; j < NR; j++) o.v[j] = row_lds[wid][row * 32 + LG * j + l];
    };
    auto dot8 = [&](const Ops &o) {
        float ax = 0.f, ay = 0.f, az = 0.f, aw = 0.f;
#pragma unroll
        for (int i = 0; i < NH; i++) {
            f16x8 h;
            __builtin_memcpy(&h, &o.hq[i], 16);
            ax = __builtin_fmaf(o.v[2 * i].x, (float)h[0], ax); ay = __builtin_fmaf(o.v[2 * i].y, (float)h[1], ay);
            az = __builtin_fmaf(o.v[2 * i].z, (float)h[2], az); aw = __builtin_fmaf(o.v[2 * i].w, (float)h[3], aw);
            ax = __builtin_fmaf(o.v[2 * i + 1].x, (float)h[4], ax); ay = __builtin_fmaf(o.v[2 * i + 1].y, (float)h[5], ay);
            az = __builtin_fmaf(o.v[2 * i + 1].z, (float)h[6], az); aw = __builtin_fmaf(o.v[2 * i + 1].w, (float)h[7], aw);
        }
        return group_sum<LG>((ax + ay) + (az + aw));
    };
    auto stash = [&](float s, uint32_t row, uint32_t, uint64_t slot, bool valid) {
        if (l == nst) { my_s = s; my_row = row; my_slot = slot; my_on = valid; }
        if (++nst == (uint32_t)LG) flush();
    };
    auto pack = [](uint32_t rl, uint32_t b, uint64_t slot) { return slot | ((uint64_t)b << 36) | ((uint64_t)rl << 60); };
    if (P <= CAP) {
        uint64_t *list = pair_list[wid];
#pragma unroll
        for (int j = 0; j < ZH_SCAN_NE; j++) {
            const uint32_t e = lane + 64u * j, c = eC[j];
            if (c) {
                const uint32_t rl = e / T, gb = eGb[j];
                {
                    const uint64_t slot = eK0[j] + eWithin[j];
                    list[off[j]] = pack(rl, eB0[j], slot);
                }
                for (uint32_t sidx = 1; sidx < c; sidx++) {
                    const ZhGroup *gp = groups + gb + sidx / GRP;
                    const uint64_t slot = gp->key_off[sidx % GRP] + eWithin[j];
                    list[off[j] + sidx] = pack(rl, gp->b[sidx % GRP], slot);
                }
            }
        }
        __builtin_amdgcn_fence(__ATOMIC_RELEASE, "wavefront");
        __builtin_amdgcn_wave_barrier();
        auto r_row = [](uint64_t r) { return (uint32_t)(r >> 60); };
        auto r_b = [](uint64_t r) { return (uint32_t)(r >> 36) & 0xFFFFFFu; };
        uint64_t rec = list[g < P ? g : P - 1];
        Ops cur;
        fetch(r_row(rec), r_b(rec), cur);
        for (uint32_t p = 0; p < P; p += G) {
            const uint32_t pn = p + G + g;
            const uint64_t recn = list[pn < P ? pn : P - 1];
            Ops nxt;
            fetch(r_row(recn), r_b(recn), nxt);
            const float s = dot8(cur);
            stash(s, r_row(rec), r_b(rec), rec & 0xFFFFFFFFFull, p + g < P);
            rec = recn; cur = nxt;
        }
    } else {
#pragma unroll
        for (int j = 0; j < ZH_SCAN_NE; j++) {
            unsigned long long m = __ballot(eC[j] != 0);
            while (m) {
                const int ll = __builtin_ctzll(m);
                m &= m - 1;
                const uint32_t c = (uint32_t)__builtin_amdgcn_readlane((int)eC[j], ll);
                const uint32_t gb = (uint32_t)__builtin_amdgcn_readlane((int)eGb[j], ll);
                const uint32_t w = (uint32_t)__builtin_amdgcn_readlane((int)eWithin[j], ll);
                const uint32_t rl = ((uint32_t)ll + 64u * j) / T;
                for (uint32_t s0 = 0; s0 < c; s0 += G) {
                    const uint32_t sidx = s0 + g < c ? s0 + g : c - 1;
                    const ZhGroup *gp = groups + gb + sidx / GRP;
                    const uint32_t b = gp->b[sidx % GRP];
                    Ops o;
                    fetch(rl, b, o);
                    const float s = dot8(o);
                    stash(s, rl, b, gp->key_off[sidx % GRP] + w, s0 + g < c);
                }
            }
        }
    }
    flush();
}

template <int D, int G>
static hipError_t launch_scan_approx_d(const float *dX, uint64_t n_rows, const ZhApprox &ap, const uint2 *dRowLeaf, uint32_t T,
                                       const uint32_t *dVisitBits, const uint4 *dNodeVisit, const ZhGroup *dGroups, uint32_t group,
                                       int metric, int mode, hipStream_t s) {
    const uint32_t RW = zh_scan_rows_per_wave(T);
    uint64_t rows_per_launch = zh_sweep_rows_per_launch(D);
    rows_per_launch = rows_per_launch / (4 * RW) * (4 * RW);
    const float Kc = zh_approx_bound(metric, D, 0);
    const int kinda = metric == ZH_COSINE ? (mode == ZH_COSINE_PARITY ? 2 : 1) : 0;
    for (uint64_t r = 0; r < n_rows; r += rows_per_launch) {
        const uint64_t r_end = r + rows_per_launch < n_rows ? r + rows_per_launch : n_rows;
        const uint64_t waves = (r_end - r + RW - 1) / RW, blocks = (waves + 3) / 4;
        if (blocks > 0x7FFFFFFFull) return hipErrorInvalidValue;
#define ZH_APX_LAUNCH(KA) \
        hipLaunchKernelGGL((scan_approx_kernel<D, G, KA>), dim3((uint32_t)blocks), dim3(256), 0, s, dX, (const uint4 *)ap.Qh, ap.qmeta, dRowLeaf, T, \
                           RW, dVisitBits, dNodeVisit, dGroups, group, r, r_end, Kc, ap.iv)
        if (kinda == 0) ZH_APX_LAUNCH(0);
        else if (kinda == 1) ZH_APX_LAUNCH(1);
        else ZH_APX_LAUNCH(2);
#undef ZH_APX_LAUNCH
    }
    return hipGetLastError();
}

bool zh_scan_mfma_supported(uint32_t d, uint32_t T) { return (d == 256 || d == 384 || d == 512 || d == 768 || d == 1024) && zh_scan_rows_per_wave(T) == 16; }
bool zh_scan_approx_supported(uint32_t d, uint32_t T, int metric) {
    if (metric != ZH_L2 && metric != ZH_L2SQ && metric != ZH_COSINE) return false;
    return zh_approx_groups(d) != 0 && zh_scan_rows_per_wave(T) != 0;
}

hipError_t zh_launch_scan_approx(const float *dX, uint32_t d, uint64_t n_rows, ZhApprox ap, const uint2 *dRowLeaf, uint32_t T,
                                 const uint32_t *dVisitBits, const uint4 *dNodeVisit, const ZhGroup *dGroups, uint32_t group, int metric,
                                 int mode, hipStream_t s) {
    if (!n_rows) return hipSuccess;
    if (ap.mfma) switch (d) {
    case 256: return launch_scan_mfma_d<256>(dX, n_rows, ap, dRowLeaf, T, dVisitBits, dNodeVisit, dGroups, group, s);
    case 384: return launch_scan_mfma_d<384>(dX, n_rows, ap, dRowLeaf, T, dVisitBits, dNodeVisit, dGroups, group, s);
    case 512: return launch_scan_mfma_d<512>(dX, n_rows, ap, dRowLeaf, T, dVisitBits, dNodeVisit, dGroups, group, s);
    case 768: return launch_scan_mfma_d<768>(dX, n_rows, ap, dRowLeaf, T, dVisitBits, dNodeVisit, dGroups, group, s);
    case 1024: return launch_scan_mfma_d<1024>(dX, n_rows, ap, dRowLeaf, T, dVisitBits, dNodeVisit, dGroups, group, s);
    default: return hipErrorInvalidValue;
    }
    switch (d) {
    case 128: {
        const uint32_t RW = zh_scan_rows_per_wave(T);
        uint64_t rows_per_launch = zh_sweep_rows_per_launch(128);
        rows_per_launch = rows_per_launch / (4 * RW) * (4 * RW);
        const float Kc = zh_approx_bound(metric, 128, 0);
        const int kinda = metric == ZH_COSINE ? (mode == ZH_COSINE_PARITY ? 2 : 1) : 0;
        for (uint64_t r = 0; r < n_rows; r += rows_per_launch) {
            const uint64_t r_end = r + rows_per_launch < n_rows ? r + rows_per_launch : n_rows;
            const uint64_t waves = (r_end - r + RW - 1) / RW, blocks = (waves + 3) / 4;
            if (blocks > 0x7FFFFFFFull) return hipErrorInvalidValue;
#define ZH_APX_LAUNCH(KA) \
            hipLaunchKernelGGL((scan_approx128_kernel<ZH_APX_G128, KA>), dim3((uint32_t)blocks), dim3(256), 0, s, dX, (const uint4 *)ap.Qh, ap.qmeta, dRowLeaf, T, RW, \
                               dVisitBits, dNodeVisit, dGroups, group, r, r_end, Kc, ap.iv)
            if (kinda == 0) ZH_APX_LAUNCH(0);
            else if (kinda == 1) ZH_APX_LAUNCH(1);
            else ZH_APX_LAUNCH(2);
#undef ZH_APX_LAUNCH
        }
        return hipGetLastError();
    }
    case 256: return launch_scan_approx_d<256, 4>(dX, n_rows, ap, dRowLeaf, T, dVisitBits, dNodeVisit, dGroups, group, metric, mode, s);
    case 384: return launch_scan_approx_d<384, 4>(dX, n_rows, ap, dRowLeaf, T, dVisitBits, dNodeVisit, dGroups, group, metric, mode, s);
    case 512: return launch_scan_approx_d<512, 2>(dX, n_rows, ap, dRowLeaf, T, dVisitBits, dNodeVisit, dGroups, group, metric, mode, s);
    case 768: return launch_scan_approx_d<768, ZH_APX_G768>(dX, n_rows, ap, dRowLeaf, T, dVisitBits, dNodeVisit, dGroups, group, metric, mode, s);
    case 1024: return launch_scan_approx_d<1024, 2>(dX, n_rows, ap, dRowLeaf, T, dVisitBits, dNodeVisit, dGroups, group, metric, mode, s);
    default: return hipErrorInvalidValue;
    }
}

#define ZH_APX_RADIX_SELECT(n, need_in, VAL, result)                                                        \
    {                                                                                                       \
        uint32_t prefix_ = 0, need_ = (need_in);                                                            \
        for (int sh_ = 24; sh_ >= 0; sh_ -= 8) {                                                            \
            __syncthreads();                                                                                \
            hist[tid] = 0;                                                                                  \
            __syncthreads();                                                                                \
            const uint32_t himask_ = sh_ == 24 ? 0u : (0xFFFFFFFFu << (sh_ + 8));                           \
            for (uint32_t i_ = tid; i_ < (n); i_ += 256) {                                                  \
                const uint32_t x_ = (VAL(i_));                                                              \
                if ((x_ & himask_) == prefix_) atomicAdd(&hist[(x_ >> sh_) & 255u], 1u);                    \
            }                                                                                               \
            __syncthreads();                                                                                \
            if (tid < 64) {                            \
                const uint32_t h0_ = hist[4 * tid], h1_ = hist[4 * tid + 1], h2_ = hist[4 * tid + 2], h3_ = hist[4 * tid + 3]; \
                const uint32_t ss_ = h0_ + h1_ + h2_ + h3_;                                                 \
                uint32_t inc_ = ss_;                                                                        \
                for (int m_ = 1; m_ < 64; m_ <<= 1) {                                                       \
                    const uint32_t t_ = __shfl_up(inc_, m_);                                                \
                    if ((int)tid >= m_) inc_ += t_;                                                         \
                }                                                                                           \
                const uint32_t exc_ = inc_ - ss_;                                                           \
                if (exc_ < need_ && need_ <= inc_) {                                                        \
                    uint32_t c_ = exc_, j_ = 4 * tid;                                                       \
                    if (need_ > c_ + h0_) { c_ += h0_; j_++;                                                \
                        if (need_ > c_ + h1_) { c_ += h1_; j_++;                                            \
                            if (need_ > c_ + h2_) { c_ += h2_; j_++; } } }                                  \
                    s_u[6] = j_; s_u[7] = c_;                                                               \
                }                                                                                           \
            }                                                                                               \
            __syncthreads();                                                                                \
            prefix_ |= s_u[6] << sh_;                                                                       \
            need_ -= s_u[7];                                                                                \
        }                                                                                                   \
        (result) = prefix_;                                                                                 \
    }

template <int KINDA>
__global__ __launch_bounds__(256) void select_tau_kernel(const ZhVisit *__restrict__ visits, uint64_t n_visits, uint32_t chunk,
                                                          uint32_t k_top, float Kc, ZhApprox ap) {
    __shared__ uint32_t hist[256];
    __shared__ uint32_t s_u[8];
    const uint32_t tid = threadIdx.x;
    const uint64_t base = (uint64_t)blockIdx.x * chunk;
    const uint32_t cnt = (uint32_t)(n_visits - base < chunk ? n_visits - base : chunk);
    for (uint32_t c = 0; c < cnt; c++) {
        const ZhVisit v = visits[base + c];
        if (v.take) {
            const float4 qm = ap.qmeta[v.b];
            uint64_t *__restrict__ raw = ap.iv + v.row_off;
            for (uint32_t i = tid; i < v.len; i += 256) {
                const uint64_t w = raw[i];
                raw[i] = approx_interval<KINDA>(__uint_as_float((uint32_t)w), __uint_as_float((uint32_t)(w >> 32)), qm, Kc, ap.row_rho, ap.rho_norm);
            }
            __syncthreads();
        }
        uint32_t tau = 0xFFFFFFFFu;
        if (v.take && v.take < v.len) {
            if (v.take < k_top) {
                if (tid == 0) {
                    const uint32_t slot = atomicAdd(&ap.ctl[0], 1u);
                    const uint32_t eb = atomicAdd(&ap.ctl[2], v.len);
                    if (slot >= ap.ex_cap) atomicOr(&ap.ctl[1], 4u);
                    else if ((uint64_t)eb + v.len > ap.ex_rows_cap) { atomicOr(&ap.ctl[1], 8u); ap.ex_visits[slot] = make_uint2(0xFFFFFFFFu, 0u); }
                    else ap.ex_visits[slot] = make_uint2((uint32_t)(base + c), eb);
                    ap.tauv[base + c] = 0u;
                }
                continue;
            }
            const uint64_t *__restrict__ kp = ap.iv + v.row_off;
#define ZH_APX_HI(i) ((uint32_t)(kp[i] >> 32))
            ZH_APX_RADIX_SELECT(v.len, v.take, ZH_APX_HI, tau);
#undef ZH_APX_HI
            if (tid == 0) atomicMin(&ap.qtau[v.b], tau);
        }
        if (tid == 0) ap.tauv[base + c] = tau;
    }
}

// ... 346 lines not shown
```

### zebra_amd/csrc/zh_internal.h

```cpp
#pragma once
#include <hip/hip_runtime.h>
#include <stddef.h>
#include <stdint.h>

#include "../../include/zebra_hip.h"

int zh_set_error(int code, const char *fmt, ...) __attribute__((format(printf, 2, 3)));
double zh_index_visits_per_pair(zh_index *ix);
void zh_search_ctx_abandon(zh_search_ctx *c);
void zh_search_ctx_stream_ordered(zh_search_ctx *c);

struct ZhVisit {
    uint32_t b;
    uint32_t leaf_off;
    uint32_t len;
    uint32_t take;
    uint64_t row_off;
    uint64_t cand_off;
    uint32_t node;
    uint32_t pad;
};

#define ZH_GROUP_MAX 4
struct ZhGroup {
// ... 44 lines not shown
    const uint32_t *leaf_ids;
    uint32_t n_nodes, n_planes, n_trees;
    uint32_t group;
};

#if defined(__HIPCC__)
__device__ __forceinline__ bool zh_plane_above(const float *__restrict__ w, float c, const float *__restrict__ x,
                                               uint32_t d) {
    float acc = 0.0f;
    if ((d & 3u) == 0) {
        const float4 *w4 = reinterpret_cast<const float4 *>(w);
        const float4 *x4 = reinterpret_cast<const float4 *>(x);
        const uint32_t n4 = d / 4;
        uint32_t k = 0;
        for (; k + 8 <= n4; k += 8) {
            float4 a[8], b[8];
#pragma unroll
            for (int u = 0; u < 8; u++) { a[u] = w4[k + u]; b[u] = x4[k + u]; }
#pragma unroll
            for (int u = 0; u < 8; u++) {
                acc = __builtin_fmaf(a[u].x, b[u].x, acc);
                acc = __builtin_fmaf(a[u].y, b[u].y, acc);
                acc = __builtin_fmaf(a[u].z, b[u].z, acc);
                acc = __builtin_fmaf(a[u].w, b[u].w, acc);
            }
        }
        for (; k < n4; k++) {
            float4 a = w4[k], b = x4[k];
            acc = __builtin_fmaf(a.x, b.x, acc);
            acc = __builtin_fmaf(a.y, b.y, acc);
            acc = __builtin_fmaf(a.z, b.z, acc);
            acc = __builtin_fmaf(a.w, b.w, acc);
        }
    } else {
        for (uint32_t k = 0; k < d; k++) acc = __builtin_fmaf(w[k], x[k], acc);
    }
    return ((double)acc + (double)c) >= 0.0;
}
#endif

#define ZH_INLINE_VISITS 32

hipError_t zh_launch_hash_dense(const float *dQ, uint32_t B, const float *dPlanes, const float *dConsts,
                                uint32_t P, uint32_t d, uint32_t *dBits, uint32_t words_per_q, float *dDots,
                                hipStream_t s);
hipError_t zh_launch_qnorm(const float *dQ, uint32_t B, uint32_t d, float *dQQ, hipStream_t s);
hipError_t zh_launch_walk_count(ZhForestDev f, const float *dQ, uint32_t B, uint32_t d, int32_t n,
                                const uint32_t *dBits, uint32_t words_per_q, uint32_t P_dense, ZhPairCounts *dCounts,
                                ZhVisit *dInline, uint32_t *dLeafCount, ZhWalkLog log, hipStream_t s);
hipError_t zh_launch_walk_blocked(ZhForestDev f, ZhBlocksDev blk, uint32_t B, int32_t n, const uint32_t *dBits,
                                  uint32_t words_per_q, ZhPairCounts *dCounts, ZhVisit *dInline, uint32_t *dLeafCount,
                                  ZhWalkLog log, const uint32_t *dUnc , const float *dQ,
                                  uint32_t d, hipStream_t s);
hipError_t zh_launch_expand(ZhForestDev f, uint32_t B, const ZhPairCounts *dCounts, const ZhVisit *dInline,
                            const uint64_t *dRowBase, const uint64_t *dCandBase, const uint64_t *dVisitBase,
                            ZhVisit *dVisits, const uint32_t *dLeafCount, uint32_t *dLeafFill,
                            const uint32_t *dGroupBase, const uint64_t *dGroupRowBase, ZhGroup *dGroups,
                            uint64_t *dGroupRowOff, ZhWalkLog log, hipStream_t s);
hipError_t zh_launch_batch_init(uint32_t *dLeafCount, uint32_t *dLeafFill, uint32_t n_nodes, ZhLogCtl *dLogCtl,
                                ZhTotals *dTotals, hipStream_t s);
hipError_t zh_launch_leaf_scan(ZhForestDev f, const uint32_t *dLeafCount, uint32_t *dGroupBase,
                               uint64_t *dGroupRowBase, ZhTotals *dTotals, hipStream_t s);
hipError_t zh_launch_pair_scan(const ZhPairCounts *dCounts, uint32_t n_pairs, uint64_t *dRowBase,
                               uint64_t *dCandBase, uint64_t *dVisitBase, ZhTotals *dTotals, const ZhLogCtl *dLogCtl,
                               hipStream_t s);
hipError_t zh_launch_walk_emit(ZhForestDev f, const float *dQ, uint32_t B, uint32_t d, int32_t n,
                               const uint32_t *dBits, uint32_t words_per_q, uint32_t P_dense,
                               const ZhPairCounts *dCounts, const ZhVisit *dInline, const uint64_t *dRowBase,
                               const uint64_t *dCandBase, const uint64_t *dVisitBase, ZhVisit *dVisits,
                               const uint32_t *dLeafCount, uint32_t *dLeafFill, const uint32_t *dGroupBase,
                               const uint64_t *dGroupRowBase, ZhGroup *dGroups, uint64_t *dGroupRowOff, hipStream_t s);
hipError_t zh_launch_sweep(const float *dX, uint32_t d, const float *dQ, const float *dQQ, const ZhGroup *dGroups,
                           const uint64_t *dGroupRowOff, uint64_t n_groups, const uint32_t *dWaveGroup,
                           const uint32_t *dLeafIds, uint64_t R_grouped, int metric, int mode, uint64_t *dKeys,
                           hipStream_t s, const uint32_t *dRunIf = nullptr);
bool zh_sweep_has_predicate(uint32_t d, int metric);
hipError_t zh_launch_wave_groups(const ZhGroup *dGroups, const uint64_t *dGroupRowOff, uint64_t n_groups, uint32_t *dWaveGroup,
                                 hipStream_t s);
#define ZH_SCAN_NE 4
bool zh_scan_sweep_supported(uint32_t d, uint32_t T, int metric);
uint32_t zh_scan_rows_per_wave(uint32_t T);
hipError_t zh_launch_row_leaf(const int4 *dNodePack, const uint32_t *dNodeTree, uint32_t n_nodes, const uint32_t *dLeafIds,
                              uint32_t T, uint64_t n_rows, uint2 *dRowLeaf, hipStream_t s);
hipError_t zh_launch_node_visits(const uint32_t *dLeafCount, const uint32_t *dGroupBase, const ZhGroup *dGroups, uint32_t n_nodes,
                                 uint32_t *dBits, uint4 *dNodeVisit, hipStream_t s);
hipError_t zh_launch_scan_sweep(const float *dX, uint32_t d, uint64_t n_rows, const float *dQ, const float *dQQ,
                                const uint2 *dRowLeaf, uint32_t T, const uint32_t *dVisitBits, const uint4 *dNodeVisit,
                                const ZhGroup *dGroups, uint32_t group, int metric, int param, uint64_t *dKeys,
                                const uint32_t *dRunIf , hipStream_t s);
uint64_t zh_sweep_rows_per_launch(uint32_t d);
hipError_t zh_launch_select(const ZhVisit *dVisits, uint64_t n_visits, const uint32_t *dLeafIds,
                            const uint64_t *dKeys, uint64_t *dCandKeys, uint32_t *dCandIds, uint32_t max_leaf_len,
                            const uint32_t *dRunIf, hipStream_t s);
hipError_t zh_launch_final(const uint64_t *dCandBase, uint32_t B, uint32_t T, uint32_t k, const uint64_t *dCandKeys,
                           const uint32_t *dCandIds, uint64_t id_base, uint64_t *dOutIds, uint64_t *dOutKeys,
                           uint32_t *dOutCounts, const uint32_t *dRunIf, hipStream_t s);
hipError_t zh_launch_merge(uint32_t S, uint32_t B, uint32_t k, const uint64_t *dIds, const uint64_t *dKeys,
                           const uint32_t *dCounts, uint64_t *dOutIds, uint64_t *dOutKeys, uint32_t *dOutCounts,
                           uint64_t stride64, uint64_t stride32, hipStream_t s);
#define ZH_DISTANCE_SCRATCH_BYTES (sizeof(ZhGroup) + 16)
hipError_t zh_launch_distance_rows(const float *dX, uint64_t n, uint32_t d, const float *dq, int metric, int mode,
                                   uint64_t *dKeys, void *dScratch, hipStream_t s);

#define ZH_APX_CTL_WORDS 8
struct ZhApprox {
    const void *Qh;
    const float4 *qmeta;
    uint64_t *iv;
    uint32_t *list_lo, *list_hi, *list_id;
    uint32_t *qcount;
    uint32_t capq;
    uint32_t *tauv;
    uint32_t *qtau;
    uint2 *ex_visits;
    uint32_t ex_cap;
    uint64_t *ex_keys, *ex_ckeys;
    uint32_t *ex_cids;
    uint32_t ex_rows_cap;
    uint32_t *ctl;
    const void *row_half;
    const float2 *row_meta;
    float row_rho;
    float rho_norm;
    uint32_t mfma;
    uint32_t n_queries;
    uint64_t iv_cap;
    float nx_max;
};
uint32_t zh_approx_groups(uint32_t d);
bool zh_approx_pays(uint32_t d);
float zh_approx_bound(int metric, uint32_t d, int mfma);
bool zh_scan_mfma_supported(uint32_t d, uint32_t T);
hipError_t zh_launch_row_half(const float *dX, uint64_t row0, uint64_t n_rows, uint32_t d, void *dXh, float2 *dRowMeta, uint32_t *dRhoMax,
                              const uint32_t *dPerm , uint64_t perm_rows, hipStream_t s);
hipError_t zh_launch_scan_order(const uint2 *dRowLeaf, uint64_t n_rows, uint32_t T, uint32_t n_keys, uint32_t *dPerm, hipStream_t s);
hipError_t zh_launch_order_agreement(const uint2 *dRowLeaf, const uint32_t *dPerm, uint64_t n_rows, uint32_t T, unsigned long long *dOut, hipStream_t s);
hipError_t zh_launch_permute_row_leaf(const uint2 *dRowLeaf, const uint32_t *dPerm, uint64_t perm_rows, uint64_t n_rows, uint32_t T, uint2 *dOut, hipStream_t s);
bool zh_scan_approx_supported(uint32_t d, uint32_t T, int metric);
hipError_t zh_launch_qhalf(const float *dQ, uint32_t B, uint32_t d, void *dQh, float4 *dQmeta, int layout, hipStream_t s);
hipError_t zh_launch_absmax(const float *dX, uint64_t n, uint32_t *dOut, hipStream_t s);
hipError_t zh_launch_row_half128(const float *dX, uint64_t row0, uint64_t n_rows, float sigma, void *dXh, uint32_t *dRhoMax, hipStream_t s);
hipError_t zh_launch_sweep128h(const void *dXh, const void *dQh, float inv, const ZhGroup *dGroups, const uint64_t *dGroupRowOff, uint64_t n_groups,
                               const uint32_t *dWaveGroup, const uint32_t *dLeafIds, uint64_t R_grouped, uint64_t *dIv, hipStream_t s,
                               const ZhApprox *fuse = nullptr, int fuse_kinda = 0, uint32_t k_top = 0, float Kc = 0.f, bool byte_rows = false);
uint64_t zh_sweep128h_rows_per_launch(bool lean, bool byte_rows);
hipError_t zh_launch_row_byte128(const float *dX, uint64_t row0, uint64_t n_rows, void *dXb, uint32_t *dNotBytes, hipStream_t s);
hipError_t zh_launch_exact_register(const ZhVisit *dVisits, uint64_t n_visits, uint32_t k, ZhApprox ap, hipStream_t s);
hipError_t zh_launch_scan_approx(const float *dX, uint32_t d, uint64_t n_rows, ZhApprox ap, const uint2 *dRowLeaf, uint32_t T,
                                 const uint32_t *dVisitBits, const uint4 *dNodeVisit, const ZhGroup *dGroups, uint32_t group, int metric,
                                 int mode, hipStream_t s);
hipError_t zh_launch_select_interval(const ZhVisit *dVisits, uint64_t n_visits, uint32_t k, const uint32_t *dLeafIds, ZhApprox ap,
                                     int metric, int mode, uint32_t d, hipStream_t s);
hipError_t zh_launch_final_interval(const ZhVisit *dVisits, const float *dX, uint32_t d, const float *dQ, const float *dQQ, uint32_t B,
                                    uint32_t k, const uint32_t *dLeafIds, int metric, int mode, uint64_t id_base, ZhApprox ap,
                                    uint64_t *dOutIds, uint64_t *dOutKeys, uint32_t *dOutCounts, uint32_t max_leaf_len, hipStream_t s);

hipError_t zh_launch_exact_score(const float *dX, uint32_t d, const uint32_t *dLive, uint64_t p0, uint32_t nr, const float *dQ,
                                 const float *dQQ, uint32_t B, int metric, int param, uint64_t *dKeys, uint64_t ld, hipStream_t s);
hipError_t zh_launch_exact_visits(uint32_t B, uint32_t nsub, uint32_t nr, uint32_t L, uint32_t k, uint64_t p0, uint64_t ld, ZhVisit *dVisits,
                                  uint64_t *dCandBase, hipStream_t s);
struct ZhExact2 {
    const void *Xh; const float2 *rowMeta; const uint32_t *perm; uint64_t perm_rows; const uint32_t *liveBits;
    const void *Qh; const float4 *qmeta; uint32_t B; float Kc, rho;
    uint32_t *tau, *cnt, *lid, *llo, *lhi; uint32_t cap; uint32_t *over;
};
bool zh_exact_mfma_supported(uint32_t d, int metric);
hipError_t zh_launch_exact_mfma(uint32_t d, int metric, int mode, const ZhExact2 &e, uint64_t p_begin, uint64_t p_end, hipStream_t s,
                                bool filtered = false);
hipError_t zh_launch_exact_prune(const ZhExact2 &e, uint32_t k, uint32_t *dScratch, hipStream_t s);
hipError_t zh_launch_exact_survivor_keys(const float *dX, uint32_t d, const float *dQ, const float *dQQ, int metric, int mode, const ZhExact2 &e,
                                         uint64_t *dCKeys, uint32_t *dCIds, hipStream_t s);
hipError_t zh_launch_exact_empty(uint32_t B, uint32_t k, uint64_t *dIds, uint64_t *dKeys, uint32_t *dCounts, hipStream_t s);

#define ZH_FILTER_BLOCK_ROWS 8192u
hipError_t zh_launch_filter_and(const uint32_t *dFilter, uint64_t n_bits, const uint32_t *dLiveBits, uint64_t n_rows, uint32_t *dOut,
                                uint32_t *dBlockCount, uint32_t *dBlockExcl, uint32_t *dScanTmp, uint32_t *dTiles, hipStream_t s);
hipError_t zh_launch_filter_permute(const uint32_t *dBits, const uint32_t *dPerm, uint64_t perm_rows, uint64_t n_rows, uint32_t *dOut,
                                    uint32_t *dBlockCount, uint32_t *dBlockExcl, uint32_t *dScanTmp, uint32_t *dTiles, hipStream_t s);
hipError_t zh_launch_filter_list(const uint32_t *dBits, uint64_t n_rows, const uint32_t *dBlockExcl, uint32_t *dList, hipStream_t s);

hipError_t zh_launch_range_collect(const uint64_t *dKeys, uint64_t ld, const uint32_t *dLive, uint64_t p0, uint32_t nr, uint32_t B,
                                   const uint64_t *dMaxKeys, uint32_t *dCnt, unsigned long long *dHitCtr, uint64_t *dPoolV, uint64_t *dPoolK,
                                   uint64_t pool_cap, hipStream_t s);
hipError_t zh_launch_range_tau(const uint64_t *dMaxKeys, uint32_t B, int metric, int mode, uint32_t *dTau, hipStream_t s);
hipError_t zh_launch_range_mfma(uint32_t d, int metric, int mode, const ZhExact2 &e, uint64_t p_begin, uint64_t p_end, uint64_t *dCand, uint64_t cand_cap,
                                unsigned long long *dCandCtr, hipStream_t s);
hipError_t zh_launch_range_survivors(const float *dX, uint32_t d, const float *dQ, const float *dQQ, int metric, int mode, const uint64_t *dCand,
                                     const unsigned long long *dCandCtr, uint64_t cand_cap, const uint64_t *dMaxKeys, uint32_t *dCnt,
                                     unsigned long long *dHitCtr, uint64_t *dPoolV, uint64_t *dPoolK, uint64_t pool_cap, hipStream_t s);
hipError_t zh_launch_range_offsets(const uint32_t *dCnt, uint32_t B, uint64_t base, uint64_t *dOff, hipStream_t s);
hipError_t zh_launch_range_sort(uint64_t *dV[2], uint64_t *dK[2], uint64_t n, uint64_t n_rows, uint32_t B, void *dTmp, size_t *tmp_bytes, uint64_t id_base,
                                uint64_t *dOutIds, uint64_t *dOutKeys, hipStream_t s);

#define ZH_JOIN_CHUNK 64u
#define ZH_JOIN_PANEL_ROWS 16384u
hipError_t zh_launch_join_gather(const float *dX, uint32_t d, const uint32_t *dRows, uint32_t B, float *dQ, hipStream_t s);
hipError_t zh_launch_join_collect(const uint64_t *dKeys, uint64_t ld, const uint32_t *dLive, uint64_t p0, uint32_t nr, const uint32_t *dQRows, uint32_t B,
                                  uint64_t max_key, unsigned long long *dHitCtr, uint64_t *dPoolV, uint64_t *dPoolK, uint64_t pool_cap, hipStream_t s);
hipError_t zh_launch_join_prep(const float2 *dRowMeta, const uint32_t *dPerm, uint64_t perm_rows, const uint32_t *dLiveBits, uint64_t n_rows, float rho,
                               float4 *dQm, uint32_t *dCid, hipStream_t s);
uint64_t zh_join_geometry(uint64_t T, uint64_t tileA0, uint64_t tileA1, uint32_t *first);
hipError_t zh_launch_join_mfma(uint32_t d, int metric, int mode, const void *dXh, const float2 *dRowMeta, const float4 *dQm, const uint32_t *dCid,
                               uint64_t n_rows, uint64_t tileA0, const uint32_t *dFirst, uint32_t n_ab, uint32_t blocks, float Kc, float rho,
                               const uint32_t *dTau, uint64_t *dCand, uint64_t cand_cap, unsigned long long *dCandCtr, hipStream_t s);
hipError_t zh_launch_join_survivors(const float *dX, uint32_t d, int metric, int mode, const uint64_t *dCand, const unsigned long long *dCandCtr,
                                    uint64_t cand_cap, uint64_t max_key, unsigned long long *dHitCtr, uint64_t *dPoolV, uint64_t *dPoolK, uint64_t pool_cap,
                                    hipStream_t s);
hipError_t zh_launch_join_panel_rows(const uint32_t *dCid, uint64_t p_begin, uint64_t p_end, uint32_t *dList, unsigned long long *dCount, hipStream_t s);
hipError_t zh_launch_join_sort(uint64_t *dV[2], uint64_t *dK[2], uint64_t n, uint64_t n_rows, void *dTmp, size_t *tmp_bytes, uint64_t id_base, uint64_t *dOutA,
                               uint64_t *dOutB, uint64_t *dOutKeys, hipStream_t s);

#define ZH_KNN_PANEL_ROWS 1024u
#define ZH_KNN_CHUNK 64u
static_assert(ZH_KNN_PANEL_ROWS % 64 == 0, "a held block is four tiles of 16 lines");
hipError_t zh_launch_knn_rowpos(const uint32_t *dCid, uint64_t n_pos, uint32_t *dPos, hipStream_t s);
hipError_t zh_launch_knn_panel(uint32_t d, const void *dXh, const float2 *dRowMeta, const uint32_t *dPos, const uint32_t *dRows, uint32_t B, void *dA,
                               float2 *dPMeta, uint32_t *dPid, hipStream_t s);
uint32_t zh_knn_chunk(uint64_t tiles, uint32_t n_ab);
hipError_t zh_launch_knn_mfma(uint32_t d, int metric, int mode, const ZhExact2 &e, const float4 *dQm, const uint32_t *dCid, uint64_t p_begin, uint64_t p_end,
                              const void *dA, const float2 *dPMeta, const uint32_t *dPid, hipStream_t s);
hipError_t zh_launch_knn_emit(const uint64_t *dInIds, const uint64_t *dInKeys, const uint32_t *dInCounts, uint32_t w, const uint32_t *dRows, uint32_t B,
                              uint64_t id_base, uint64_t first_row, uint32_t k, uint64_t *dOutIds, uint64_t *dOutKeys, uint32_t *dOutCounts, hipStream_t s);

#define ZH_FKNN_SLAB 65536u
#define ZH_FKNN_HELD_ROWS 4096u
#define ZH_FKNN_COL_TILES 2048u
#define ZH_FKNN_CHUNK 64u
static_assert(ZH_FKNN_HELD_ROWS % 64 == 0, "a held block is four tiles of 16 lines");
struct ZhFknnSeg {
    uint32_t col0, ct;
    uint32_t held_off, held_len;
    uint32_t line0, held_tiles;
// ... 134 lines not shown
```

### zebra_amd/csrc/zh_search.hip

```cpp
#include <cstdlib>

#include "zh_internal.h"
#include "zh_device.h"

#define HD_KT 32
#define HD_PITCH 65

template <bool WRITE_DOTS>
__global__ __launch_bounds__(256) void hash_dense_kernel(const float *__restrict__ Q, uint32_t B,
                                                          const float *__restrict__ W,
                                                          const float *__restrict__ C, uint32_t P, uint32_t d,
                                                          uint32_t *__restrict__ bits, uint32_t wpq,
                                                          float *__restrict__ dots) {
    __shared__ float Qs[HD_KT][HD_PITCH];
    __shared__ float Ws[HD_KT][HD_PITCH];
    const uint32_t tid = threadIdx.x, lane = tid & 63, wv = tid >> 6;
    const uint32_t wr = wv >> 1, wc = wv & 1;
    const uint32_t p0 = blockIdx.x * 64, b0 = blockIdx.y * 64;
    f32x16 acc;
#pragma unroll
    for (int i = 0; i < 16; i++) acc[i] = 0.0f;
    const bool vec4 = (d & 3u) == 0;
    auto fetch = [&](uint32_t k0, float4 *qv, float4 *wv) {
#pragma unroll
// ... 1447 lines not shown
    }
    return hipGetLastError();
}

template <int KIND>
static hipError_t launch_sweep_kind(const SweepArgs &a) {
#define ZH_SWEEP_CASE(DD) case DD: return launch_sweep_k<DD, KIND>(a)
    if constexpr (KIND == K_L2 || KIND == K_COS) {
        switch (a.d) {
            ZH_SWEEP_CASE(64);
            ZH_SWEEP_CASE(256);
            ZH_SWEEP_CASE(512);
            ZH_SWEEP_CASE(1024);
            ZH_SWEEP_CASE(1536);
        default: break;
        }
    }
    switch (a.d) {
        ZH_SWEEP_CASE(128);
        ZH_SWEEP_CASE(384);
        ZH_SWEEP_CASE(768);
    default: return launch_sweep_k<0, KIND>(a);
    }
#undef ZH_SWEEP_CASE
}

bool zh_sweep_has_predicate(uint32_t d, int metric) {
    const int kind = zh_kind_of(metric);
    return d == 128 && (kind == K_L2 || kind == K_COS);
}

uint32_t zh_group_size(uint32_t dim) {
    return 4u;
}

hipError_t zh_launch_sweep(const float *dX, uint32_t d, const float *dQ, const float *dQQ, const ZhGroup *dGroups,
                           const uint64_t *dGroupRowOff, uint64_t n_groups, const uint32_t *dWaveGroup,
                           const uint32_t *dLeafIds, uint64_t R_grouped, int metric, int param, uint64_t *dKeys,
                           hipStream_t s, const uint32_t *dRunIf) {
    if (R_grouped == 0 || n_groups == 0) return hipSuccess;
    if (dRunIf && !zh_sweep_has_predicate(d, metric)) return hipErrorInvalidValue;
    const SweepArgs a{dX, d, dQ, dQQ, dGroups, dGroupRowOff, n_groups, dWaveGroup, dLeafIds, R_grouped, metric, param, dKeys, s, dRunIf};
#define ZH_KIND_CASE(K) case K: return launch_sweep_kind<K>(a)
    switch (zh_kind_of(metric)) {
        ZH_KIND_CASE(K_COS);
        ZH_KIND_CASE(K_MAX);
        ZH_KIND_CASE(K_CANB);
        ZH_KIND_CASE(K_BRAY);
        ZH_KIND_CASE(K_ABS);
        ZH_KIND_CASE(K_P3);
        ZH_KIND_CASE(K_P4);
        ZH_KIND_CASE(K_HAMM);
        ZH_KIND_CASE(K_PP);
    default: return launch_sweep_kind<K_L2>(a);
    }
#undef ZH_KIND_CASE
}

__global__ __launch_bounds__(64) void row_leaf_kernel(const int4 *__restrict__ node_pack, const uint32_t *__restrict__ node_tree,
                                                       const uint32_t *__restrict__ leaf_ids, uint32_t T, uint64_t n_rows,
                                                       uint32_t node0, uint2 *__restrict__ rowLeaf) {
    const uint32_t node = node0 + blockIdx.x;
    const int4 rec = node_pack[node];
    if (rec.x >= 0) return;
    const uint32_t t = node_tree[node];
    if (t >= T) return;
    const uint32_t off = (uint32_t)rec.y, len = (uint32_t)rec.z;
    for (uint32_t i = threadIdx.x; i < len; i += 64) {
        const uint32_t r = leaf_ids[(size_t)off + i];
        if (r < n_rows) rowLeaf[(size_t)r * T + t] = make_uint2(node, i);
    }
}
hipError_t zh_launch_row_leaf(const int4 *dNodePack, const uint32_t *dNodeTree, uint32_t n_nodes, const uint32_t *dLeafIds,
                              uint32_t T, uint64_t n_rows, uint2 *dRowLeaf, hipStream_t s) {
    hipError_t e = hipMemsetAsync(dRowLeaf, 0xFF, n_rows * T * sizeof(uint2), s);
    if (e != hipSuccess) return e;
    for (uint32_t n0 = 0; n0 < n_nodes; n0 += (1u << 22)) {
        const uint32_t nb = n_nodes - n0 < (1u << 22) ? n_nodes - n0 : (1u << 22);
        hipLaunchKernelGGL(row_leaf_kernel, dim3(nb), dim3(64), 0, s, dNodePack, dNodeTree, dLeafIds, T, n_rows, n0, dRowLeaf);
    }
    return hipGetLastError();
}

__global__ __launch_bounds__(256) void node_visit_kernel(const uint32_t *__restrict__ leafCount, const uint32_t *__restrict__ groupBase,
                                                          const ZhGroup *__restrict__ groups, uint32_t n_nodes,
                                                          uint32_t *__restrict__ bits, uint4 *__restrict__ nodeVisit) {
    const uint32_t w = blockIdx.x * blockDim.x + threadIdx.x;
    const uint32_t n0 = w * 32;
    if (n0 >= n_nodes) return;
    uint32_t word = 0;
    for (uint32_t i = 0; i < 32 && n0 + i < n_nodes; i++) {
        const uint32_t c = leafCount[n0 + i];
        if (c) {
            word |= 1u << i;
            const uint32_t gb = groupBase[n0 + i];
            const uint64_t k0 = groups[gb].key_off[0];
            nodeVisit[n0 + i] = make_uint4(c | ((uint32_t)(k0 >> 32) << 28), gb, groups[gb].b[0], (uint32_t)k0);
        }
    }
    bits[w] = word;
}
hipError_t zh_launch_node_visits(const uint32_t *dLeafCount, const uint32_t *dGroupBase, const ZhGroup *dGroups, uint32_t n_nodes,
                                 uint32_t *dBits, uint4 *dNodeVisit, hipStream_t s) {
    const uint32_t words = (n_nodes + 31) / 32;
    if (!words) return hipSuccess;
    hipLaunchKernelGGL(node_visit_kernel, dim3((words + 255) / 256), dim3(256), 0, s, dLeafCount, dGroupBase, dGroups, n_nodes, dBits, dNodeVisit);
    return hipGetLastError();
}

#define ZH_SCAN_CAP 256
template <int D, int KIND>
__global__ __launch_bounds__(256) void scan_sweep_kernel(const float *__restrict__ X, const float *__restrict__ Q,
                                                          const float *__restrict__ QQ, const uint2 *__restrict__ rowLeaf,
                                                          uint32_t T, uint32_t RW, const uint32_t *__restrict__ visitBits,
                                                          const uint4 *__restrict__ nodeVisit,
                                                          const ZhGroup *__restrict__ groups, uint32_t GRP, uint64_t row_begin,
                                                          uint64_t row_end, int metric, int param,
                                                          uint64_t *__restrict__ keys, const uint32_t *__restrict__ run_if) {
    constexpr int NV = RowVec<D>::NV;
    __shared__ uint4 pair_list[4][ZH_SCAN_CAP];
    if (run_if && *run_if == 0) return;
    const uint32_t lane = threadIdx.x & 63;
    const uint32_t wid = (uint32_t)__builtin_amdgcn_readfirstlane((int)(threadIdx.x >> 6));
    const uint64_t wave = (uint64_t)blockIdx.x * (blockDim.x >> 6) + wid;
    const uint64_t r0 = row_begin + wave * RW;
    if (r0 >= row_end) return;
    const uint32_t nr = (uint32_t)(row_end - r0 < RW ? row_end - r0 : RW);
    const uint32_t n_ent = nr * T;
    const uint2 *__restrict__ ent = rowLeaf + (size_t)r0 * T;
    uint32_t eGb[ZH_SCAN_NE], eWithin[ZH_SCAN_NE], eC[ZH_SCAN_NE], off[ZH_SCAN_NE], eB0[ZH_SCAN_NE];
    uint64_t eK0[ZH_SCAN_NE];
    uint32_t P = 0;
#pragma unroll
    for (int j = 0; j < ZH_SCAN_NE; j++) {
        const uint32_t e = lane + 64u * j;
        eGb[j] = 0; eWithin[j] = 0; eC[j] = 0; eB0[j] = 0; eK0[j] = 0;
        if (e < n_ent) {
            const unsigned long long rlw = __builtin_nontemporal_load(reinterpret_cast<const unsigned long long *>(ent + e));
            const uint2 rl = make_uint2((uint32_t)rlw, (uint32_t)(rlw >> 32));
            eWithin[j] = rl.y;
            if (rl.x != 0xFFFFFFFFu && ((visitBits[rl.x >> 5] >> (rl.x & 31)) & 1u)) {
                const uint4 nv = nodeVisit[rl.x];
                eC[j] = nv.x & 0x0FFFFFFFu; eGb[j] = nv.y; eB0[j] = nv.z;
                eK0[j] = ((uint64_t)(nv.x >> 28) << 32) | nv.w;
            }
        }
        uint32_t incl = eC[j];
#pragma unroll
        for (int o = 1; o < 64; o <<= 1) {
            const uint32_t t = __shfl_up(incl, o);
            if (lane >= (uint32_t)o) incl += t;
        }
        off[j] = P + incl - eC[j];
        P += (uint32_t)__builtin_amdgcn_readlane((int)incl, 63);
    }
    if (P == 0) return;
    float my_s0 = 0.f, my_s1 = 0.f;
    uint64_t my_slot = 0;
    uint32_t my_b = 0, npend = 0;
    auto flush = [&]() {
        if (lane < npend) {
            uint64_t key;
            if constexpr (KIND == K_COS) key = key_cosine(my_s0, my_s1, QQ[my_b], param);
            else if constexpr (KIND == K_L2) key = key_l2(my_s0, metric);
            else key = key_of(metric, param, my_s0, my_s1, 0.f);
            __builtin_nontemporal_store(key, keys + my_slot);
        }
        npend = 0;
    };
    auto row_norm = [&](const float4 *v) {
        float4 c = make_float4(0.f, 0.f, 0.f, 0.f);
#pragma unroll
        for (int j = 0; j < NV; j++) {
            const bool act = (j < RowVec<D>::NJ) || (lane < (uint32_t)RowVec<D>::REM4);
            if (act) sq4(v[j], c);
        }
        return wave_sum_canonical((c.x + c.y) + (c.z + c.w));
    };
    auto score = [&](const float4 *v, float a2, uint32_t b, uint64_t slot, const float4 *q) {
        float s0 = 0.f, s1 = 0.f;
        row_pair_sums<D, KIND>(v, q, lane, param, s0, s1);
        if (lane == npend) { my_s0 = s0; my_s1 = KIND == K_COS ? a2 : s1; my_slot = slot; my_b = b; }
        if (++npend == 64) flush();
    };
    if (P <= ZH_SCAN_CAP) {
        uint4 *list = pair_list[wid];
        uint32_t mrows = 0;
#pragma unroll
        for (int j = 0; j < ZH_SCAN_NE; j++) {
            const uint32_t c = eC[j];
            if (c) {
                const uint32_t rl = (lane + 64u * j) / T, gb = eGb[j];
                mrows |= 1u << rl;
                {
                    const uint64_t slot = eK0[j] + eWithin[j];
                    list[off[j]] = make_uint4(rl, eB0[j], (uint32_t)slot, (uint32_t)(slot >> 32));
                }
                for (uint32_t sidx = 1; sidx < c; sidx++) {
                    const ZhGroup *g = groups + gb + sidx / GRP;
                    const uint64_t slot = g->key_off[sidx % GRP] + eWithin[j];
                    list[off[j] + sidx] = make_uint4(rl, g->b[sidx % GRP], (uint32_t)slot, (uint32_t)(slot >> 32));
                }
            }
        }
        uint32_t rowmask = 0;
#pragma unroll
        for (int bit = 0; bit < 16; bit++) rowmask |= (__ballot((mrows >> bit) & 1u) != 0 ? 1u : 0u) << bit;
        __builtin_amdgcn_fence(__ATOMIC_RELEASE, "wavefront");
        __builtin_amdgcn_wave_barrier();
        auto rd = [&](uint32_t p) {
            const uint4 r = list[p];
            return make_uint4((uint32_t)__builtin_amdgcn_readfirstlane((int)r.x), (uint32_t)__builtin_amdgcn_readfirstlane((int)r.y),
                              (uint32_t)__builtin_amdgcn_readfirstlane((int)r.z), (uint32_t)__builtin_amdgcn_readfirstlane((int)r.w));
        };
        float4 qa[NV], qb[NV], qc[NV], qd[NV];
        uint32_t p = 0;
        auto segment = [&](const float4 *vr, float a2, uint32_t rowid) {
            for (;;) {
                const uint4 ra = rd(p < P ? p : P - 1), rb = rd(p + 1 < P ? p + 1 : P - 1), rc = rd(p + 2 < P ? p + 2 : P - 1),
                            rdd = rd(p + 3 < P ? p + 3 : P - 1);
                const bool ha = p < P && ra.x == rowid, hb = ha && p + 1 < P && rb.x == rowid, hc = hb && p + 2 < P && rc.x == rowid,
                           hd = hc && p + 3 < P && rdd.x == rowid;
                if (!ha) return;
                load_row<D>(Q + (size_t)ra.y * D, lane, qa);
                if (hb) load_row<D>(Q + (size_t)rb.y * D, lane, qb);
                if (hc) load_row<D>(Q + (size_t)rc.y * D, lane, qc);
                if (hd) load_row<D>(Q + (size_t)rdd.y * D, lane, qd);
                score(vr, a2, ra.y, ((uint64_t)ra.w << 32) | ra.z, qa);
                if (hb) score(vr, a2, rb.y, ((uint64_t)rb.w << 32) | rb.z, qb);
                if (hc) score(vr, a2, rc.y, ((uint64_t)rc.w << 32) | rc.z, qc);
                if (hd) score(vr, a2, rdd.y, ((uint64_t)rdd.w << 32) | rdd.z, qd);
                p += hd ? 4u : (hc ? 3u : (hb ? 2u : 1u));
                if (!hd) return;
            }
        };
        while (rowmask) {
            uint32_t rid[4];
#pragma unroll
            for (int r = 0; r < 4; r++) {
                rid[r] = rowmask ? (uint32_t)__builtin_ctz(rowmask) : 0xFFFFFFFFu;
                rowmask &= rowmask - 1;
            }
            float4 v0[NV], v1[NV], v2[NV], v3[NV];
            load_row<D, true>(X + (size_t)(r0 + rid[0]) * D, lane, v0);
            if (rid[1] != 0xFFFFFFFFu) load_row<D, true>(X + (size_t)(r0 + rid[1]) * D, lane, v1);
            if (rid[2] != 0xFFFFFFFFu) load_row<D, true>(X + (size_t)(r0 + rid[2]) * D, lane, v2);
            if (rid[3] != 0xFFFFFFFFu) load_row<D, true>(X + (size_t)(r0 + rid[3]) * D, lane, v3);
            segment(v0, KIND == K_COS ? row_norm(v0) : 0.f, rid[0]);
            if (rid[1] != 0xFFFFFFFFu) segment(v1, KIND == K_COS ? row_norm(v1) : 0.f, rid[1]);
            if (rid[2] != 0xFFFFFFFFu) segment(v2, KIND == K_COS ? row_norm(v2) : 0.f, rid[2]);
            if (rid[3] != 0xFFFFFFFFu) segment(v3, KIND == K_COS ? row_norm(v3) : 0.f, rid[3]);
        }
    } else {
        float4 v[NV];
        float a2 = 0.f;
        uint32_t cur = 0xFFFFFFFFu;
#pragma unroll
        for (int j = 0; j < ZH_SCAN_NE; j++) {
            unsigned long long m = __ballot(eC[j] != 0);
            while (m) {
                const int l = __builtin_ctzll(m);
                m &= m - 1;
                const uint32_t c = (uint32_t)__builtin_amdgcn_readlane((int)eC[j], l);
                const uint32_t gb = (uint32_t)__builtin_amdgcn_readlane((int)eGb[j], l);
                const uint32_t w = (uint32_t)__builtin_amdgcn_readlane((int)eWithin[j], l);
                const uint32_t rl = ((uint32_t)l + 64u * j) / T;
                if (rl != cur) {
                    cur = rl;
                    load_row<D, true>(X + (size_t)(r0 + rl) * D, lane, v);
                    if (KIND == K_COS) a2 = row_norm(v);
                }
                for (uint32_t sidx = 0; sidx < c; sidx++) {
                    const ZhGroup *g = groups + gb + sidx / GRP;
                    const uint32_t b = g->b[sidx % GRP];
                    float4 q[NV];
                    load_row<D>(Q + (size_t)b * D, lane, q);
                    score(v, a2, b, g->key_off[sidx % GRP] + w, q);
                }
            }
        }
    }
    flush();
}

#define ZH_SCAN128_CAP 192
template <int KIND>
__global__ __launch_bounds__(256) void scan128_sweep_kernel(const float *__restrict__ X, const float *__restrict__ Q,
                                                             const float *__restrict__ QQ, const uint2 *__restrict__ rowLeaf,
                                                             uint32_t T, uint32_t RW, const uint32_t *__restrict__ visitBits,
                                                             const uint4 *__restrict__ nodeVisit,
                                                             const ZhGroup *__restrict__ groups, uint32_t GRP, uint64_t row_begin,
                                                             uint64_t row_end, int metric, int param,
                                                             uint64_t *__restrict__ keys, const uint32_t *__restrict__ run_if) {
    static_assert(KIND == K_L2 || KIND == K_COS, "the paired scan covers the two simsimd-path kinds");
    if (run_if && *run_if == 0) return;
    __shared__ uint4 pair_list[4][ZH_SCAN128_CAP];
    __shared__ float4 row_lds[4][4][32];
    __shared__ uint32_t row_start[4][20];
    const uint32_t lane = threadIdx.x & 63, hl = lane & 31, half = lane >> 5;
    const uint32_t wid = (uint32_t)__builtin_amdgcn_readfirstlane((int)(threadIdx.x >> 6));
    const uint64_t wave = (uint64_t)blockIdx.x * (blockDim.x >> 6) + wid;
    const uint64_t r0 = row_begin + wave * RW;
    if (r0 >= row_end) return;
    const uint32_t nr = (uint32_t)(row_end - r0 < RW ? row_end - r0 : RW);
    const uint32_t n_ent = nr * T;
    const uint2 *__restrict__ ent = rowLeaf + (size_t)r0 * T;
    const float4 *__restrict__ X4 = reinterpret_cast<const float4 *>(X);
    const float4 *__restrict__ Q4 = reinterpret_cast<const float4 *>(Q);
    uint32_t eGb[ZH_SCAN_NE], eWithin[ZH_SCAN_NE], eC[ZH_SCAN_NE], off[ZH_SCAN_NE], eB0[ZH_SCAN_NE];
    uint64_t eK0[ZH_SCAN_NE];
    uint32_t P = 0;
#pragma unroll
    for (int j = 0; j < ZH_SCAN_NE; j++) {
        const uint32_t e = lane + 64u * j;
        eGb[j] = 0; eWithin[j] = 0; eC[j] = 0; eB0[j] = 0; eK0[j] = 0;
        if (e < n_ent) {
            const unsigned long long rlw = __builtin_nontemporal_load(reinterpret_cast<const unsigned long long *>(ent + e));
            const uint2 rl = make_uint2((uint32_t)rlw, (uint32_t)(rlw >> 32));
            eWithin[j] = rl.y;
            if (rl.x != 0xFFFFFFFFu && ((visitBits[rl.x >> 5] >> (rl.x & 31)) & 1u)) {
                const uint4 nv = nodeVisit[rl.x];
                eC[j] = nv.x & 0x0FFFFFFFu; eGb[j] = nv.y; eB0[j] = nv.z;
                eK0[j] = ((uint64_t)(nv.x >> 28) << 32) | nv.w;
            }
        }
        uint32_t incl = eC[j];
#pragma unroll
        for (int o = 1; o < 64; o <<= 1) {
            const uint32_t t = __shfl_up(incl, o);
            if (lane >= (uint32_t)o) incl += t;
        }
        off[j] = P + incl - eC[j];
        P += (uint32_t)__builtin_amdgcn_readlane((int)incl, 63);
    }
    if (P == 0) return;
    float my_s0 = 0.f, my_s1 = 0.f;
    uint64_t my_slot = ~0ull;
    uint32_t my_b = 0;
    if (P <= ZH_SCAN128_CAP) {
        uint4 *list = pair_list[wid];
        uint32_t *rstart = row_start[wid];
#pragma unroll
        for (int j = 0; j < ZH_SCAN_NE; j++) {
            const uint32_t e = lane + 64u * j, c = eC[j];
            if (e < n_ent && e % T == 0) rstart[e / T] = off[j];
            if (c) {
                const uint32_t rl = e / T, gb = eGb[j];
                {
                    const uint64_t slot = eK0[j] + eWithin[j];
                    list[off[j]] = make_uint4(rl, eB0[j], (uint32_t)slot, (uint32_t)(slot >> 32));
                }
                for (uint32_t sidx = 1; sidx < c; sidx++) {
                    const ZhGroup *g = groups + gb + sidx / GRP;
                    const uint64_t slot = g->key_off[sidx % GRP] + eWithin[j];
                    list[off[j] + sidx] = make_uint4(rl, g->b[sidx % GRP], (uint32_t)slot, (uint32_t)(slot >> 32));
                }
            }
        }
        if (lane == 0) rstart[nr] = P;
        __builtin_amdgcn_fence(__ATOMIC_RELEASE, "wavefront");
        __builtin_amdgcn_wave_barrier();
        uint32_t npl = 0;
        auto flush = [&]() {
            if (hl < npl && my_slot != ~0ull)
                __builtin_nontemporal_store(key_of(metric, param, my_s0, my_s1, KIND == K_COS ? QQ[my_b] : 0.f), keys + my_slot);
            npl = 0;
        };
        for (uint32_t rb = 0; rb < nr; rb += 4) {
            const uint32_t re = rb + 4 < nr ? rb + 4 : nr;
            const uint32_t pa = (uint32_t)__builtin_amdgcn_readfirstlane((int)rstart[rb]);
            const uint32_t pb = (uint32_t)__builtin_amdgcn_readfirstlane((int)rstart[re]);
            if (pa == pb) continue;
            {
                const uint32_t ra = rb + half, rc = rb + 2 + half;
                float4 va = make_float4(0.f, 0.f, 0.f, 0.f), vc = va;
                if (ra < re) va = ld16<true>(X4 + (size_t)(r0 + ra) * 32 + hl);
                if (rc < re) vc = ld16<true>(X4 + (size_t)(r0 + rc) * 32 + hl);
                row_lds[wid][half][hl] = va;
                row_lds[wid][2 + half][hl] = vc;
            }
            __builtin_amdgcn_fence(__ATOMIC_RELEASE, "wavefront");
            __builtin_amdgcn_wave_barrier();
            uint32_t pi = pa + half;
            uint4 rec = list[pi < pb ? pi : pb - 1];
            float4 qc = Q4[(size_t)rec.y * 32 + hl];
            for (uint32_t p = pa; p < pb; p += 2) {
                const bool valid = p + half < pb;
                const uint32_t pn = p + 2 + half;
                const uint4 recn = list[pn < pb ? pn : pb - 1];
                const float4 qn = Q4[(size_t)recn.y * 32 + hl];
                const float4 v = row_lds[wid][rec.x - rb][hl];
                float a2 = 0.f;
                if (KIND == K_COS) {
                    float4 c;
                    c.x = __builtin_fmaf(v.x, v.x, 0.f); c.y = __builtin_fmaf(v.y, v.y, 0.f);
                    c.z = __builtin_fmaf(v.z, v.z, 0.f); c.w = __builtin_fmaf(v.w, v.w, 0.f);
                    a2 = half_sum_canonical((c.x + c.y) + (c.z + c.w));
                }
                float4 a = make_float4(0.f, 0.f, 0.f, 0.f), e1 = a;
                acc4<KIND>(v, qc, a, e1, param);
                const float s0 = half_sum_canonical((a.x + a.y) + (a.z + a.w));
                if (hl == npl) {
                    my_s0 = s0; my_s1 = a2; my_b = rec.y;
                    my_slot = valid ? (((uint64_t)rec.w << 32) | rec.z) : ~0ull;
                }
                if (++npl == 32) flush();
                rec = recn; qc = qn;
            }
            __builtin_amdgcn_wave_barrier();
        }
        flush();
        return;
    }
    uint32_t npend = 0;
    auto flush1 = [&]() {
        if (lane < npend) __builtin_nontemporal_store(key_of(metric, param, my_s0, my_s1, KIND == K_COS ? QQ[my_b] : 0.f), keys + my_slot);
        npend = 0;
    };
    float4 v[1];
    float a2 = 0.f;
    uint32_t cur = 0xFFFFFFFFu;
#pragma unroll
    for (int j = 0; j < ZH_SCAN_NE; j++) {
        unsigned long long m = __ballot(eC[j] != 0);
        while (m) {
            const int l = __builtin_ctzll(m);
            m &= m - 1;
            const uint32_t c = (uint32_t)__builtin_amdgcn_readlane((int)eC[j], l);
            const uint32_t gb = (uint32_t)__builtin_amdgcn_readlane((int)eGb[j], l);
            const uint32_t w = (uint32_t)__builtin_amdgcn_readlane((int)eWithin[j], l);
            const uint32_t rl = ((uint32_t)l + 64u * j) / T;
            if (rl != cur) {
                cur = rl;
                load_row<128, true>(X + (size_t)(r0 + rl) * 128, lane, v);
                if (KIND == K_COS) {
                    float4 c4 = make_float4(0.f, 0.f, 0.f, 0.f);
                    if (lane < 32) {
                        c4.x = __builtin_fmaf(v[0].x, v[0].x, 0.f); c4.y = __builtin_fmaf(v[0].y, v[0].y, 0.f);
                        c4.z = __builtin_fmaf(v[0].z, v[0].z, 0.f); c4.w = __builtin_fmaf(v[0].w, v[0].w, 0.f);
                    }
                    a2 = wave_sum_canonical((c4.x + c4.y) + (c4.z + c4.w));
                }
            }
            for (uint32_t sidx = 0; sidx < c; sidx++) {
                const ZhGroup *g = groups + gb + sidx / GRP;
                const uint32_t b = g->b[sidx % GRP];
                float4 q[1];
                load_row<128>(Q + (size_t)b * 128, lane, q);
                float s0 = 0.f, s1 = 0.f;
                row_pair_sums<128, KIND>(v, q, lane, param, s0, s1);
                if (lane == npend) { my_s0 = s0; my_s1 = KIND == K_COS ? a2 : s1; my_slot = g->key_off[sidx % GRP] + w; my_b = b; }
                if (++npend == 64) flush1();
            }
        }
    }
    flush1();
}

uint32_t zh_scan_rows_per_wave(uint32_t T) {
    if (T == 0 || T > 64u * ZH_SCAN_NE) return 0;
    const uint32_t rw = 64u * ZH_SCAN_NE / T;
    return rw > 16 ? 16 : rw;
}
bool zh_scan_sweep_supported(uint32_t d, uint32_t T, int metric) {
    if (!zh_scan_rows_per_wave(T)) return false;
    const int kind = zh_kind_of(metric);
    if (d == 128 || d == 384 || d == 768) return true;
    if (kind != K_L2 && kind != K_COS) return false;
    switch (d) { case 64: case 256: case 512: case 1024: case 1536: return true; default: return false; }
}

template <int D, int KIND>
static hipError_t launch_scan_dk(const float *dX, uint64_t n_rows, const float *dQ, const float *dQQ, const uint2 *dRowLeaf,
                                 uint32_t T, const uint32_t *dVisitBits, const uint4 *dNodeVisit, const ZhGroup *dGroups,
                                 uint32_t group, int metric, int param, uint64_t *dKeys, const uint32_t *dRunIf, hipStream_t s) {
    const uint32_t RW = zh_scan_rows_per_wave(T);
    uint64_t rows_per_launch = zh_sweep_rows_per_launch(D);
    rows_per_launch = rows_per_launch / (4 * RW) * (4 * RW);
    for (uint64_t r = 0; r < n_rows; r += rows_per_launch) {
        const uint64_t r_end = r + rows_per_launch < n_rows ? r + rows_per_launch : n_rows;
        const uint64_t waves = (r_end - r + RW - 1) / RW, blocks = (waves + 3) / 4;
        if (blocks > 0x7FFFFFFFull) return hipErrorInvalidValue;
        if constexpr (D == 128 && (KIND == K_L2 || KIND == K_COS))
            hipLaunchKernelGGL((scan128_sweep_kernel<KIND>), dim3((uint32_t)blocks), dim3(256), 0, s, dX, dQ, dQQ, dRowLeaf, T, RW,
                               dVisitBits, dNodeVisit, dGroups, group, r, r_end, metric, param, dKeys, dRunIf);
        else
            hipLaunchKernelGGL((scan_sweep_kernel<D, KIND>), dim3((uint32_t)blocks), dim3(256), 0, s, dX, dQ, dQQ, dRowLeaf, T, RW,
                               dVisitBits, dNodeVisit, dGroups, group, r, r_end, metric, param, dKeys, dRunIf);
    }
    return hipGetLastError();
}
template <int KIND>
static hipError_t launch_scan_k(const float *dX, uint32_t d, uint64_t n_rows, const float *dQ, const float *dQQ,
                                const uint2 *dRowLeaf, uint32_t T, const uint32_t *dVisitBits, const uint4 *dNodeVisit,
                                const ZhGroup *dGroups, uint32_t group, int metric, int param, uint64_t *dKeys, const uint32_t *dRunIf, hipStream_t s) {
#define ZH_SCAN_CASE(DD) \
    case DD: return launch_scan_dk<DD, KIND>(dX, n_rows, dQ, dQQ, dRowLeaf, T, dVisitBits, dNodeVisit, dGroups, group, metric, param, dKeys, dRunIf, s)
    if constexpr (KIND == K_L2 || KIND == K_COS) {
        switch (d) {
            ZH_SCAN_CASE(64); ZH_SCAN_CASE(256); ZH_SCAN_CASE(512); ZH_SCAN_CASE(1024); ZH_SCAN_CASE(1536);
        default: break;
        }
    }
    switch (d) {
        ZH_SCAN_CASE(128); ZH_SCAN_CASE(384); ZH_SCAN_CASE(768);
    default: return hipErrorInvalidValue;
    }
#undef ZH_SCAN_CASE
}
hipError_t zh_launch_scan_sweep(const float *dX, uint32_t d, uint64_t n_rows, const float *dQ, const float *dQQ,
                                const uint2 *dRowLeaf, uint32_t T, const uint32_t *dVisitBits, const uint4 *dNodeVisit,
                                const ZhGroup *dGroups, uint32_t group, int metric, int param, uint64_t *dKeys, const uint32_t *dRunIf,
                                hipStream_t s) {
    if (!n_rows) return hipSuccess;
#define ZH_KIND_CASE(K) \
    case K: return launch_scan_k<K>(dX, d, n_rows, dQ, dQQ, dRowLeaf, T, dVisitBits, dNodeVisit, dGroups, group, metric, param, dKeys, dRunIf, s)
    switch (zh_kind_of(metric)) {
        ZH_KIND_CASE(K_COS);
        ZH_KIND_CASE(K_MAX);
        ZH_KIND_CASE(K_CANB);
        ZH_KIND_CASE(K_BRAY);
        ZH_KIND_CASE(K_ABS);
        ZH_KIND_CASE(K_P3);
        ZH_KIND_CASE(K_P4);
        ZH_KIND_CASE(K_HAMM);
        ZH_KIND_CASE(K_PP);
    default: return launch_scan_k<K_L2>(dX, d, n_rows, dQ, dQQ, dRowLeaf, T, dVisitBits, dNodeVisit, dGroups, group, metric, param, dKeys, dRunIf, s);
    }
#undef ZH_KIND_CASE
}

__global__ void one_group_kernel(ZhGroup *g, uint64_t *rowoff, uint64_t n) {
    g->leaf_off = 0; g->len = (uint32_t)n; g->gsize = 1; g->take4 = 0;
    for (int m = 0; m < ZH_GROUP_MAX; m++) { g->b[m] = 0; g->key_off[m] = 0; }
    rowoff[0] = 0;
}
hipError_t zh_launch_distance_rows(const float *dX, uint64_t n, uint32_t d, const float *dq, int metric, int mode,
                                   uint64_t *dKeys, void *dScratch, hipStream_t s) {
    if (!n) return hipSuccess;
    ZhGroup *dg = reinterpret_cast<ZhGroup *>(dScratch);
    uint64_t *dro = reinterpret_cast<uint64_t *>(dg + 1);
    float *dqq = reinterpret_cast<float *>(dro + 1);
    hipLaunchKernelGGL(one_group_kernel, dim3(1), dim3(1), 0, s, dg, dro, n);
    hipError_t e = zh_launch_qnorm(dq, 1, d, dqq, s);
    if (e == hipSuccess) e = zh_launch_sweep(dX, d, dq, dqq, dg, dro, 1, nullptr, nullptr, n, metric, mode, dKeys, s);
    return e;
}

#define SEL_GROUP_LEN 16
template <int CAP>
__global__ __launch_bounds__(256) void select_kernel(const ZhVisit *__restrict__ visits, uint64_t n_visits, uint32_t chunk,
                                                      const uint32_t *__restrict__ leaf_ids,
                                                      const uint64_t *__restrict__ keys,
                                                      uint64_t *__restrict__ cand_keys,
                                                      uint32_t *__restrict__ cand_ids, const uint32_t *__restrict__ run_if) {
    __shared__ uint64_t sk[CAP];
    __shared__ __attribute__((aligned(16))) uint32_t si[CAP < 2048 ? 2048 : CAP];
    __shared__ uint32_t s_u32[8];
    __shared__ uint32_t s_list[256], s_small[256], s_nlist, s_nsmall;
    const uint32_t tid = threadIdx.x;
    if (run_if && *run_if == 0) return;
    const uint64_t base = (uint64_t)blockIdx.x * chunk;
    const uint32_t cnt = (uint32_t)(n_visits - base < chunk ? n_visits - base : chunk);
    if (tid == 0) { s_nlist = 0; s_nsmall = 0; }
    __syncthreads();
    if (tid < cnt) {
        const uint32_t len = visits[base + tid].len, take = visits[base + tid].take;
        if (take > 0) {
            if (len <= SEL_GROUP_LEN) s_small[atomicAdd(&s_nsmall, 1u)] = tid;
            else s_list[atomicAdd(&s_nlist, 1u)] = tid;
        }
    }
    __syncthreads();
    {
        const uint32_t ns = s_nsmall, g = tid >> 4, l = tid & 15;
        for (uint32_t i = g; i < ns; i += 16) {
            const ZhVisit v = visits[base + s_small[i]];
            const bool on = l < v.len;
            const uint64_t k = on ? keys[v.row_off + l] : ~0ull;
            const uint32_t id = on ? leaf_ids[(size_t)v.leaf_off + l] : ~0u;
            uint32_t rank = l;
            if (v.take < v.len) {
                rank = 0;
#pragma unroll
                for (int j = 0; j < SEL_GROUP_LEN; j++) {
                    const uint64_t kj = __shfl(k, j, SEL_GROUP_LEN);
                    const uint32_t ij = __shfl(id, j, SEL_GROUP_LEN);
                    rank += (kj < k || (kj == k && ij < id)) ? 1u : 0u;
                }
            }
            if (on && rank < v.take) {
                cand_keys[v.cand_off + rank] = k;
                cand_ids[v.cand_off + rank] = id;
            }
        }
    }
    const uint32_t nl = s_nlist;
    for (uint32_t li = 0; li < nl; li++) {
        const ZhVisit v = visits[base + s_list[li]];
        if (v.take >= v.len) {
            for (uint32_t i = tid; i < v.len; i += 256) {
                cand_keys[v.cand_off + i] = keys[v.row_off + i];
                cand_ids[v.cand_off + i] = leaf_ids[(size_t)v.leaf_off + i];
            }
            continue;
        }
        bool need_slow = false;
        if (v.len <= CAP) select_fast<true>(v, leaf_ids, keys, cand_keys, cand_ids, sk, si, s_u32, need_slow);
        else select_fast<false>(v, leaf_ids, keys, cand_keys, cand_ids, sk, si, s_u32, need_slow);
        if (need_slow) {
// ... 528 lines not shown
```

Baseline: 203,200.

## Compact node visit records with rank-indexed bitmap words

Replaces the dense per-node visit record array, which had one uint4 per tree node, with a compact array holding only visited nodes. It is indexed through bitmap words that carry a prefix count, and the rank is computed with popcount. This shrinks the record buffer and the memory footprint it touches when few nodes are visited, which should improve cache locality in the scan kernels. In exchange it adds a second counting kernel launch for the block prefix sums and a dependent popcount/rank step on each lookup.

```diff
diff --git a/zebra_amd/csrc/zh_api.hip b/zebra_amd/csrc/zh_api.hip
--- a/zebra_amd/csrc/zh_api.hip
+++ b/zebra_amd/csrc/zh_api.hip
@@ -97,7 +97,7 @@
 struct zh_search_ctx {
     zh_index *ix = nullptr;
     DevBuf wQQ, wBits, wCounts, wInline, wRowBase, wCandBase, wVisitBase, wTotals, wVisits, wKeys, wCandKeys, wCandIds,
-        wLeafCount, wLeafFill, wGroupBase, wGroupRowBase, wGroups, wGroupRowOff, wWaveGroup, wVisitBits, wNodeVisit, wScore, wJunkBits, wZeros, wQnorm, wQpad, wFixList, wLogPool, wLogHead, wLogCtl,
+        wLeafCount, wLeafFill, wGroupBase, wGroupRowBase, wGroups, wGroupRowOff, wWaveGroup, wVisitWords, wVisitRec, wScore, wJunkBits, wZeros, wQnorm, wQpad, wFixList, wLogPool, wLogHead, wLogCtl,
         wPfRows, wPfCounts, wPfKeys, wPfIds, wPfAmb, wPfCtl, wUnc, wQh, wQmeta, wApList, wApCount, wApEx, wApExKeys, wApCtl, wRaw;
     ZhApprox dbg_ap{};
     bool dbg_valid = false, dbg_raw = false;
@@ -134,7 +134,7 @@
     hipStream_t sv_heavy = nullptr;
     std::vector<DevBuf *> all_bufs() {
         return {&wQQ, &wBits, &wCounts, &wInline, &wRowBase, &wCandBase, &wVisitBase, &wTotals, &wVisits, &wKeys,
-                &wCandKeys, &wCandIds, &wLeafCount, &wLeafFill, &wGroupBase, &wGroupRowBase, &wGroups, &wGroupRowOff, &wWaveGroup, &wVisitBits, &wNodeVisit, &wScore, &wJunkBits, &wZeros, &wQnorm, &wQpad, &wFixList,
+                &wCandKeys, &wCandIds, &wLeafCount, &wLeafFill, &wGroupBase, &wGroupRowBase, &wGroups, &wGroupRowOff, &wWaveGroup, &wVisitWords, &wVisitRec, &wScore, &wJunkBits, &wZeros, &wQnorm, &wQpad, &wFixList,
                 &wLogPool, &wLogHead, &wLogCtl, &wQwin, &wOutWin, &wPfRows, &wPfCounts, &wPfKeys, &wPfIds, &wPfAmb, &wPfCtl, &wUnc,
                 &wQh, &wQmeta, &wApList, &wApCount, &wApEx, &wApExKeys, &wApCtl, &wRaw};
     }
@@ -2383,11 +2383,10 @@
         if (!ix->row_leaf_valid || ix->row_leaf_rows != ix->n_rows) c->scan = false;
     }
     if (c->scan) {
-        const size_t nn = std::max<uint32_t>(ix->n_nodes, 1);
-        if ((rc = c->wVisitBits.ensure((nn + 31) / 32 * 4))) return rc;
-        if ((rc = c->wNodeVisit.ensure(nn * sizeof(uint4)))) return rc;
+        if ((rc = c->wVisitWords.ensure(zh_visit_words_bytes(std::max<uint32_t>(ix->n_nodes, 1))))) return rc;
+        if ((rc = c->wVisitRec.ensure(std::max<uint64_t>(std::min<uint64_t>(tot.visits, ix->n_nodes), 1) * sizeof(uint4)))) return rc;
         HIPCHK(zh_launch_node_visits(c->wLeafCount.as<uint32_t>(), c->wGroupBase.as<uint32_t>(), c->wGroups.as<ZhGroup>(), ix->n_nodes,
-                                     c->wVisitBits.as<uint32_t>(), c->wNodeVisit.as<uint4>(), s));
+                                     c->wVisitWords.as<uint2>(), c->wVisitRec.as<uint4>(), s));
     }
     if (!c->scan)
         HIPCHK(zh_launch_wave_groups(c->wGroups.as<ZhGroup>(), c->wGroupRowOff.as<uint64_t>(), tot.groups, c->wWaveGroup.as<uint32_t>(), s));
@@ -2464,11 +2463,11 @@
                                    tot.groups, c->wWaveGroup.as<uint32_t>(), f.leaf_ids, tot.group_rows, c->wKeys.as<uint64_t>(), hs,
                                    c->approx_fused ? &ap : nullptr, kinda, (uint32_t)k, zh_approx_bound(c->metric, d, 2), c->approx_bytes));
     else if (c->approx)
-        HIPCHK(zh_launch_scan_approx(ix->X.as<float>(), d, ix->n_rows, ap, mfma ? scan_row_leaf : ix->row_leaf.as<uint2>(), T, c->wVisitBits.as<uint32_t>(),
-                                     c->wNodeVisit.as<uint4>(), c->wGroups.as<ZhGroup>(), f.group, c->metric, c->mode, hs));
+        HIPCHK(zh_launch_scan_approx(ix->X.as<float>(), d, ix->n_rows, ap, mfma ? scan_row_leaf : ix->row_leaf.as<uint2>(), T, c->wVisitWords.as<uint2>(),
+                                     c->wVisitRec.as<uint4>(), c->wGroups.as<ZhGroup>(), f.group, c->metric, c->mode, hs));
     else if (c->scan)
         HIPCHK(zh_launch_scan_sweep(ix->X.as<float>(), d, ix->n_rows, c->dQ, c->wQQ.as<float>(), ix->row_leaf.as<uint2>(), T,
-                                    c->wVisitBits.as<uint32_t>(), c->wNodeVisit.as<uint4>(), c->wGroups.as<ZhGroup>(), f.group,
+                                    c->wVisitWords.as<uint2>(), c->wVisitRec.as<uint4>(), c->wGroups.as<ZhGroup>(), f.group,
                                     c->metric, c->mode, c->wKeys.as<uint64_t>(), nullptr, hs));
     else
         HIPCHK(zh_launch_sweep(ix->X.as<float>(), d, c->dQ, c->wQQ.as<float>(), c->wGroups.as<ZhGroup>(),
@@ -2499,7 +2498,7 @@
                                    c->wWaveGroup.as<uint32_t>(), f.leaf_ids, tot.group_rows, c->metric, c->mode, c->wKeys.as<uint64_t>(), s, run_if));
         else
             HIPCHK(zh_launch_scan_sweep(ix->X.as<float>(), d, ix->n_rows, c->dQ, c->wQQ.as<float>(), ix->row_leaf.as<uint2>(), T,
-                                        c->wVisitBits.as<uint32_t>(), c->wNodeVisit.as<uint4>(), c->wGroups.as<ZhGroup>(), f.group,
+                                        c->wVisitWords.as<uint2>(), c->wVisitRec.as<uint4>(), c->wGroups.as<ZhGroup>(), f.group,
                                         c->metric, c->mode, c->wKeys.as<uint64_t>(), run_if, s));
     }
     HIPCHK(zh_launch_select(c->wVisits.as<ZhVisit>(), tot.visits, f.leaf_ids, c->wKeys.as<uint64_t>(),
diff --git a/zebra_amd/csrc/zh_approx.hip b/zebra_amd/csrc/zh_approx.hip
--- a/zebra_amd/csrc/zh_approx.hip
+++ b/zebra_amd/csrc/zh_approx.hip
@@ -104,7 +104,7 @@
 
 
 __device__ __forceinline__ uint32_t scan_phase1(uint32_t lane, uint32_t n_ent, const uint2 *__restrict__ ent,
-                                                const uint32_t *__restrict__ visitBits, const uint4 *__restrict__ nodeVisit,
+                                                const uint2 *__restrict__ visitWords, const uint4 *__restrict__ visitRec,
                                                 uint32_t *eGb, uint32_t *eWithin, uint32_t *eC, uint32_t *off, uint32_t *eB0, uint64_t *eK0) {
     unsigned long long rlw[ZH_SCAN_NE];
 #pragma unroll
@@ -112,20 +112,20 @@
         const uint32_t e = lane + 64u * j;
         rlw[j] = __builtin_nontemporal_load(reinterpret_cast<const unsigned long long *>(ent + (e < n_ent ? e : 0)));
     }
-    uint32_t word[ZH_SCAN_NE];
+    uint2 word[ZH_SCAN_NE];
     bool in[ZH_SCAN_NE];
 #pragma unroll
     for (int j = 0; j < ZH_SCAN_NE; j++) {
         const uint32_t node = (uint32_t)rlw[j];
         in[j] = lane + 64u * j < n_ent && node != 0xFFFFFFFFu;
-        word[j] = visitBits[in[j] ? node >> 5 : 0];
+        word[j] = visitWords[in[j] ? node >> 5 : 0];
     }
     uint4 nv[ZH_SCAN_NE];
 #pragma unroll
     for (int j = 0; j < ZH_SCAN_NE; j++) {
         const uint32_t node = (uint32_t)rlw[j];
-        in[j] = in[j] && ((word[j] >> (node & 31)) & 1u);
-        nv[j] = nodeVisit[in[j] ? node : 0];
+        in[j] = in[j] && ((word[j].x >> (node & 31)) & 1u);
+        nv[j] = visitRec[in[j] ? word[j].y + __popc(word[j].x & ((1u << (node & 31)) - 1u)) : 0];
     }
     uint32_t P = 0;
 #pragma unroll
@@ -160,8 +160,8 @@
 #endif
 void scan_approx_kernel(const float *__restrict__ X, const uint4 *__restrict__ Qh,
                                                            const float4 *__restrict__ qmeta, const uint2 *__restrict__ rowLeaf,
-                                                           uint32_t T, uint32_t RW, const uint32_t *__restrict__ visitBits,
-                                                           const uint4 *__restrict__ nodeVisit, const ZhGroup *__restrict__ groups,
+                                                           uint32_t T, uint32_t RW, const uint2 *__restrict__ visitWords,
+                                                           const uint4 *__restrict__ visitRec, const ZhGroup *__restrict__ groups,
                                                            uint32_t GRP, uint64_t row_begin, uint64_t row_end, float Kc,
                                                            uint64_t *__restrict__ iv) {
     constexpr int LG = 64 / G, NH = D * G / 512, NR = 2 * NH;
@@ -179,7 +179,7 @@
     const uint2 *__restrict__ ent = rowLeaf + (size_t)r0 * T;
     uint32_t eGb[ZH_SCAN_NE], eWithin[ZH_SCAN_NE], eC[ZH_SCAN_NE], off[ZH_SCAN_NE], eB0[ZH_SCAN_NE];
     uint64_t eK0[ZH_SCAN_NE];
-    const uint32_t P = scan_phase1(lane, n_ent, ent, visitBits, nodeVisit, eGb, eWithin, eC, off, eB0, eK0);
+    const uint32_t P = scan_phase1(lane, n_ent, ent, visitWords, visitRec, eGb, eWithin, eC, off, eB0, eK0);
     if (P == 0) return;
     const float4 *__restrict__ X4 = reinterpret_cast<const float4 *>(X);
     float my_s = 0.f, my_a2 = 0.f;
@@ -441,8 +441,8 @@
 __global__ __launch_bounds__(256) __attribute__((amdgpu_waves_per_eu(D > 768 ? 2 : ZH_MFMA_WAVES, D > 768 ? 2 : ZH_MFMA_WAVES)))
 void scan_mfma_kernel(const u32x4v *__restrict__ Xh, const float *__restrict__ Xf, const float2 *__restrict__ rowMeta,
                                                          const uint4 *__restrict__ Qh, const uint2 *__restrict__ rowLeaf, uint32_t T,
-                                                         uint32_t RW, const uint32_t *__restrict__ visitBits,
-                                                         const uint4 *__restrict__ nodeVisit, const ZhGroup *__restrict__ groups,
+                                                         uint32_t RW, const uint2 *__restrict__ visitWords,
+                                                         const uint4 *__restrict__ visitRec, const ZhGroup *__restrict__ groups,
                                                          uint32_t GRP, uint64_t row_begin, uint64_t row_end, uint64_t *__restrict__ iv,
                                                          uint32_t *__restrict__ colStats ,
                                                          uint32_t nq, uint64_t iv_cap, uint32_t *__restrict__ guard) {
@@ -468,7 +468,7 @@
     const uint2 *__restrict__ ent = rowLeaf + (size_t)r0 * T;
     uint32_t eGb[ZH_SCAN_NE], eWithin[ZH_SCAN_NE], eC[ZH_SCAN_NE], off[ZH_SCAN_NE], eB0[ZH_SCAN_NE];
     uint64_t eK0[ZH_SCAN_NE];
-    const uint32_t P = scan_phase1(lane, n_ent, ent, visitBits, nodeVisit, eGb, eWithin, eC, off, eB0, eK0);
+    const uint32_t P = scan_phase1(lane, n_ent, ent, visitWords, visitRec, eGb, eWithin, eC, off, eB0, eK0);
     if (P == 0) return;
     SP(const uint64_t sp1 = clock64();)
     uint64_t *list = pair_list[wid];
@@ -736,7 +736,7 @@
 
 template <int D>
 static hipError_t launch_scan_mfma_d(const float *dX, uint64_t n_rows, const ZhApprox &ap, const uint2 *dRowLeaf, uint32_t T,
-                                     const uint32_t *dVisitBits, const uint4 *dNodeVisit, const ZhGroup *dGroups, uint32_t group, hipStream_t s) {
+                                     const uint2 *dVisitWords, const uint4 *dVisitRec, const ZhGroup *dGroups, uint32_t group, hipStream_t s) {
     const uint32_t RW = zh_scan_rows_per_wave(T);
     uint64_t rows_per_launch = zh_sweep_rows_per_launch(D);
     rows_per_launch = rows_per_launch / (4 * RW) * (4 * RW);
@@ -746,10 +746,10 @@
         if (blocks > 0x7FFFFFFFull) return hipErrorInvalidValue;
         if (ap.row_half)
             hipLaunchKernelGGL((scan_mfma_kernel<D, false>), dim3((uint32_t)blocks), dim3(256), 0, s, (const u32x4v *)ap.row_half, dX, ap.row_meta, (const uint4 *)ap.Qh, dRowLeaf, T, RW,
-                               dVisitBits, dNodeVisit, dGroups, group, r, r_end, ap.iv, ap.ctl + 5, ap.n_queries, ap.iv_cap, ap.ctl + 7);
+                               dVisitWords, dVisitRec, dGroups, group, r, r_end, ap.iv, ap.ctl + 5, ap.n_queries, ap.iv_cap, ap.ctl + 7);
         else
             hipLaunchKernelGGL((scan_mfma_kernel<D, true>), dim3((uint32_t)blocks), dim3(256), 0, s, (const u32x4v *)nullptr, dX, ap.row_meta, (const uint4 *)ap.Qh, dRowLeaf, T, RW,
-                               dVisitBits, dNodeVisit, dGroups, group, r, r_end, ap.iv, ap.ctl + 5, ap.n_queries, ap.iv_cap, ap.ctl + 7);
+                               dVisitWords, dVisitRec, dGroups, group, r, r_end, ap.iv, ap.ctl + 5, ap.n_queries, ap.iv_cap, ap.ctl + 7);
     }
     return hipGetLastError();
 }
@@ -1796,8 +1796,8 @@
 template <int G, int KINDA>
 __global__ __launch_bounds__(256) void scan_approx128_kernel(const float *__restrict__ X, const uint4 *__restrict__ Qh,
                                                               const float4 *__restrict__ qmeta, const uint2 *__restrict__ rowLeaf,
-                                                              uint32_t T, uint32_t RW, const uint32_t *__restrict__ visitBits,
-                                                              const uint4 *__restrict__ nodeVisit, const ZhGroup *__restrict__ groups,
+                                                              uint32_t T, uint32_t RW, const uint2 *__restrict__ visitWords,
+                                                              const uint4 *__restrict__ visitRec, const ZhGroup *__restrict__ groups,
                                                               uint32_t GRP, uint64_t row_begin, uint64_t row_end, float Kc,
                                                               uint64_t *__restrict__ iv) {
     constexpr int LG = 64 / G, NH = G / 4, NR = 2 * NH;
@@ -1815,7 +1815,7 @@
     const uint2 *__restrict__ ent = rowLeaf + (size_t)r0 * T;
     uint32_t eGb[ZH_SCAN_NE], eWithin[ZH_SCAN_NE], eC[ZH_SCAN_NE], off[ZH_SCAN_NE], eB0[ZH_SCAN_NE];
     uint64_t eK0[ZH_SCAN_NE];
-    const uint32_t P = scan_phase1(lane, n_ent, ent, visitBits, nodeVisit, eGb, eWithin, eC, off, eB0, eK0);
+    const uint32_t P = scan_phase1(lane, n_ent, ent, visitWords, visitRec, eGb, eWithin, eC, off, eB0, eK0);
     if (P == 0) return;
     {
         const float4 *src = reinterpret_cast<const float4 *>(X) + (size_t)r0 * 32;
@@ -1932,7 +1932,7 @@
 
 template <int D, int G>
 static hipError_t launch_scan_approx_d(const float *dX, uint64_t n_rows, const ZhApprox &ap, const uint2 *dRowLeaf, uint32_t T,
-                                       const uint32_t *dVisitBits, const uint4 *dNodeVisit, const ZhGroup *dGroups, uint32_t group,
+                                       const uint2 *dVisitWords, const uint4 *dVisitRec, const ZhGroup *dGroups, uint32_t group,
                                        int metric, int mode, hipStream_t s) {
     const uint32_t RW = zh_scan_rows_per_wave(T);
     uint64_t rows_per_launch = zh_sweep_rows_per_launch(D);
@@ -1945,7 +1945,7 @@
         if (blocks > 0x7FFFFFFFull) return hipErrorInvalidValue;
 #define ZH_APX_LAUNCH(KA) \
         hipLaunchKernelGGL((scan_approx_kernel<D, G, KA>), dim3((uint32_t)blocks), dim3(256), 0, s, dX, (const uint4 *)ap.Qh, ap.qmeta, dRowLeaf, T, \
-                           RW, dVisitBits, dNodeVisit, dGroups, group, r, r_end, Kc, ap.iv)
+                           RW, dVisitWords, dVisitRec, dGroups, group, r, r_end, Kc, ap.iv)
         if (kinda == 0) ZH_APX_LAUNCH(0);
         else if (kinda == 1) ZH_APX_LAUNCH(1);
         else ZH_APX_LAUNCH(2);
@@ -1961,15 +1961,15 @@
 }
 
 hipError_t zh_launch_scan_approx(const float *dX, uint32_t d, uint64_t n_rows, ZhApprox ap, const uint2 *dRowLeaf, uint32_t T,
-                                 const uint32_t *dVisitBits, const uint4 *dNodeVisit, const ZhGroup *dGroups, uint32_t group, int metric,
+                                 const uint2 *dVisitWords, const uint4 *dVisitRec, const ZhGroup *dGroups, uint32_t group, int metric,
                                  int mode, hipStream_t s) {
     if (!n_rows) return hipSuccess;
     if (ap.mfma) switch (d) {
-    case 256: return launch_scan_mfma_d<256>(dX, n_rows, ap, dRowLeaf, T, dVisitBits, dNodeVisit, dGroups, group, s);
-    case 384: return launch_scan_mfma_d<384>(dX, n_rows, ap, dRowLeaf, T, dVisitBits, dNodeVisit, dGroups, group, s);
-    case 512: return launch_scan_mfma_d<512>(dX, n_rows, ap, dRowLeaf, T, dVisitBits, dNodeVisit, dGroups, group, s);
-    case 768: return launch_scan_mfma_d<768>(dX, n_rows, ap, dRowLeaf, T, dVisitBits, dNodeVisit, dGroups, group, s);
-    case 1024: return launch_scan_mfma_d<1024>(dX, n_rows, ap, dRowLeaf, T, dVisitBits, dNodeVisit, dGroups, group, s);
+    case 256: return launch_scan_mfma_d<256>(dX, n_rows, ap, dRowLeaf, T, dVisitWords, dVisitRec, dGroups, group, s);
+    case 384: return launch_scan_mfma_d<384>(dX, n_rows, ap, dRowLeaf, T, dVisitWords, dVisitRec, dGroups, group, s);
+    case 512: return launch_scan_mfma_d<512>(dX, n_rows, ap, dRowLeaf, T, dVisitWords, dVisitRec, dGroups, group, s);
+    case 768: return launch_scan_mfma_d<768>(dX, n_rows, ap, dRowLeaf, T, dVisitWords, dVisitRec, dGroups, group, s);
+    case 1024: return launch_scan_mfma_d<1024>(dX, n_rows, ap, dRowLeaf, T, dVisitWords, dVisitRec, dGroups, group, s);
     default: return hipErrorInvalidValue;
     }
     switch (d) {
@@ -1985,7 +1985,7 @@
             if (blocks > 0x7FFFFFFFull) return hipErrorInvalidValue;
 #define ZH_APX_LAUNCH(KA) \
             hipLaunchKernelGGL((scan_approx128_kernel<ZH_APX_G128, KA>), dim3((uint32_t)blocks), dim3(256), 0, s, dX, (const uint4 *)ap.Qh, ap.qmeta, dRowLeaf, T, RW, \
-                               dVisitBits, dNodeVisit, dGroups, group, r, r_end, Kc, ap.iv)
+                               dVisitWords, dVisitRec, dGroups, group, r, r_end, Kc, ap.iv)
             if (kinda == 0) ZH_APX_LAUNCH(0);
             else if (kinda == 1) ZH_APX_LAUNCH(1);
             else ZH_APX_LAUNCH(2);
@@ -1993,11 +1993,11 @@
         }
         return hipGetLastError();
     }
-    case 256: return launch_scan_approx_d<256, 4>(dX, n_rows, ap, dRowLeaf, T, dVisitBits, dNodeVisit, dGroups, group, metric, mode, s);
-    case 384: return launch_scan_approx_d<384, 4>(dX, n_rows, ap, dRowLeaf, T, dVisitBits, dNodeVisit, dGroups, group, metric, mode, s);
-    case 512: return launch_scan_approx_d<512, 2>(dX, n_rows, ap, dRowLeaf, T, dVisitBits, dNodeVisit, dGroups, group, metric, mode, s);
-    case 768: return launch_scan_approx_d<768, ZH_APX_G768>(dX, n_rows, ap, dRowLeaf, T, dVisitBits, dNodeVisit, dGroups, group, metric, mode, s);
-    case 1024: return launch_scan_approx_d<1024, 2>(dX, n_rows, ap, dRowLeaf, T, dVisitBits, dNodeVisit, dGroups, group, metric, mode, s);
+    case 256: return launch_scan_approx_d<256, 4>(dX, n_rows, ap, dRowLeaf, T, dVisitWords, dVisitRec, dGroups, group, metric, mode, s);
+    case 384: return launch_scan_approx_d<384, 4>(dX, n_rows, ap, dRowLeaf, T, dVisitWords, dVisitRec, dGroups, group, metric, mode, s);
+    case 512: return launch_scan_approx_d<512, 2>(dX, n_rows, ap, dRowLeaf, T, dVisitWords, dVisitRec, dGroups, group, metric, mode, s);
+    case 768: return launch_scan_approx_d<768, ZH_APX_G768>(dX, n_rows, ap, dRowLeaf, T, dVisitWords, dVisitRec, dGroups, group, metric, mode, s);
+    case 1024: return launch_scan_approx_d<1024, 2>(dX, n_rows, ap, dRowLeaf, T, dVisitWords, dVisitRec, dGroups, group, metric, mode, s);
     default: return hipErrorInvalidValue;
     }
 }
diff --git a/zebra_amd/csrc/zh_internal.h b/zebra_amd/csrc/zh_internal.h
--- a/zebra_amd/csrc/zh_internal.h
+++ b/zebra_amd/csrc/zh_internal.h
@@ -150,10 +150,14 @@
 uint32_t zh_scan_rows_per_wave(uint32_t T);
 hipError_t zh_launch_row_leaf(const int4 *dNodePack, const uint32_t *dNodeTree, uint32_t n_nodes, const uint32_t *dLeafIds,
                               uint32_t T, uint64_t n_rows, uint2 *dRowLeaf, hipStream_t s);
+static inline size_t zh_visit_words_bytes(uint32_t n_nodes) {
+    const size_t words = ((size_t)n_nodes + 31) / 32;
+    return words * sizeof(uint2) + (words + 255) / 256 * sizeof(uint32_t);
+}
 hipError_t zh_launch_node_visits(const uint32_t *dLeafCount, const uint32_t *dGroupBase, const ZhGroup *dGroups, uint32_t n_nodes,
-                                 uint32_t *dBits, uint4 *dNodeVisit, hipStream_t s);
+                                 uint2 *dVisitWords, uint4 *dVisitRec, hipStream_t s);
 hipError_t zh_launch_scan_sweep(const float *dX, uint32_t d, uint64_t n_rows, const float *dQ, const float *dQQ,
-                                const uint2 *dRowLeaf, uint32_t T, const uint32_t *dVisitBits, const uint4 *dNodeVisit,
+                                const uint2 *dRowLeaf, uint32_t T, const uint2 *dVisitWords, const uint4 *dVisitRec,
                                 const ZhGroup *dGroups, uint32_t group, int metric, int param, uint64_t *dKeys,
                                 const uint32_t *dRunIf , hipStream_t s);
 uint64_t zh_sweep_rows_per_launch(uint32_t d);
@@ -215,7 +219,7 @@
 hipError_t zh_launch_row_byte128(const float *dX, uint64_t row0, uint64_t n_rows, void *dXb, uint32_t *dNotBytes, hipStream_t s);
 hipError_t zh_launch_exact_register(const ZhVisit *dVisits, uint64_t n_visits, uint32_t k, ZhApprox ap, hipStream_t s);
 hipError_t zh_launch_scan_approx(const float *dX, uint32_t d, uint64_t n_rows, ZhApprox ap, const uint2 *dRowLeaf, uint32_t T,
-                                 const uint32_t *dVisitBits, const uint4 *dNodeVisit, const ZhGroup *dGroups, uint32_t group, int metric,
+                                 const uint2 *dVisitWords, const uint4 *dVisitRec, const ZhGroup *dGroups, uint32_t group, int metric,
                                  int mode, hipStream_t s);
 hipError_t zh_launch_select_interval(const ZhVisit *dVisits, uint64_t n_visits, uint32_t k, const uint32_t *dLeafIds, ZhApprox ap,
                                      int metric, int mode, uint32_t d, hipStream_t s);
diff --git a/zebra_amd/csrc/zh_search.hip b/zebra_amd/csrc/zh_search.hip
--- a/zebra_amd/csrc/zh_search.hip
+++ b/zebra_amd/csrc/zh_search.hip
@@ -1553,38 +1553,72 @@
     return hipGetLastError();
 }
 
+__device__ __forceinline__ uint32_t visit_word(const uint32_t *__restrict__ leafCount, uint32_t w, uint32_t n_nodes) {
+    uint32_t word = 0;
+    if (w < (n_nodes + 31) / 32) {
+        const uint32_t n0 = w * 32;
+        for (uint32_t i = 0; i < 32 && i < n_nodes - n0; i++)
+            if (leafCount[n0 + i]) word |= 1u << i;
+    }
+    return word;
+}
+__global__ __launch_bounds__(256) void node_visit_count_kernel(const uint32_t *__restrict__ leafCount, uint32_t n_nodes,
+                                                                uint32_t *__restrict__ blockSum) {
+    __shared__ uint32_t s_w[4];
+    uint32_t cnt = __popc(visit_word(leafCount, blockIdx.x * blockDim.x + threadIdx.x, n_nodes));
+    for (int m = 1; m < 64; m <<= 1) cnt += __shfl_xor(cnt, m);
+    if ((threadIdx.x & 63) == 0) s_w[threadIdx.x >> 6] = cnt;
+    __syncthreads();
+    if (threadIdx.x == 0) blockSum[blockIdx.x] = s_w[0] + s_w[1] + s_w[2] + s_w[3];
+}
 __global__ __launch_bounds__(256) void node_visit_kernel(const uint32_t *__restrict__ leafCount, const uint32_t *__restrict__ groupBase,
                                                           const ZhGroup *__restrict__ groups, uint32_t n_nodes,
-                                                          uint32_t *__restrict__ bits, uint4 *__restrict__ nodeVisit) {
-    const uint32_t w = blockIdx.x * blockDim.x + threadIdx.x;
-    const uint32_t n0 = w * 32;
-    if (n0 >= n_nodes) return;
-    uint32_t word = 0;
-    for (uint32_t i = 0; i < 32 && n0 + i < n_nodes; i++) {
-        const uint32_t c = leafCount[n0 + i];
-        if (c) {
-            word |= 1u << i;
-            const uint32_t gb = groupBase[n0 + i];
-            const uint64_t k0 = groups[gb].key_off[0];
-            nodeVisit[n0 + i] = make_uint4(c | ((uint32_t)(k0 >> 32) << 28), gb, groups[gb].b[0], (uint32_t)k0);
-        }
-    }
-    bits[w] = word;
+                                                          const uint32_t *__restrict__ blockSum, uint2 *__restrict__ words,
+                                                          uint4 *__restrict__ visitRec) {
+    __shared__ uint32_t s_before[4], s_w[4];
+    const uint32_t tid = threadIdx.x, lane = tid & 63, wv = tid >> 6;
+    const uint32_t w = blockIdx.x * blockDim.x + tid;
+    uint32_t before = 0;
+    for (uint32_t b = tid; b < blockIdx.x; b += 256) before += blockSum[b];
+    for (int m = 1; m < 64; m <<= 1) before += __shfl_xor(before, m);
+    const uint32_t word = visit_word(leafCount, w, n_nodes), cnt = __popc(word);
+    uint32_t incl = cnt;
+    for (int o = 1; o < 64; o <<= 1) {
+        const uint32_t t = __shfl_up(incl, o);
+        if (lane >= (uint32_t)o) incl += t;
+    }
+    if (lane == 0) s_before[wv] = before;
+    if (lane == 63) s_w[wv] = incl;
+    __syncthreads();
+    uint32_t rank = s_before[0] + s_before[1] + s_before[2] + s_before[3] + incl - cnt;
+    for (uint32_t v = 0; v < wv; v++) rank += s_w[v];
+    if (w >= (n_nodes + 31) / 32) return;
+    words[w] = make_uint2(word, rank);
+    for (uint32_t rest = word; rest; rest &= rest - 1) {
+        const uint32_t n = w * 32 + (uint32_t)__builtin_ctz(rest);
+        const uint32_t gb = groupBase[n];
+        const uint64_t k0 = groups[gb].key_off[0];
+        visitRec[rank++] = make_uint4(leafCount[n] | ((uint32_t)(k0 >> 32) << 28), gb, groups[gb].b[0], (uint32_t)k0);
+    }
 }
 hipError_t zh_launch_node_visits(const uint32_t *dLeafCount, const uint32_t *dGroupBase, const ZhGroup *dGroups, uint32_t n_nodes,
-                                 uint32_t *dBits, uint4 *dNodeVisit, hipStream_t s) {
+                                 uint2 *dVisitWords, uint4 *dVisitRec, hipStream_t s) {
     const uint32_t words = (n_nodes + 31) / 32;
     if (!words) return hipSuccess;
-    hipLaunchKernelGGL(node_visit_kernel, dim3((words + 255) / 256), dim3(256), 0, s, dLeafCount, dGroupBase, dGroups, n_nodes, dBits, dNodeVisit);
+    uint32_t *blockSum = reinterpret_cast<uint32_t *>(dVisitWords + words);
+    const dim3 grid((words + 255) / 256);
+    hipLaunchKernelGGL(node_visit_count_kernel, grid, dim3(256), 0, s, dLeafCount, n_nodes, blockSum);
+    hipLaunchKernelGGL(node_visit_kernel, grid, dim3(256), 0, s, dLeafCount, dGroupBase, dGroups, n_nodes, blockSum, dVisitWords, dVisitRec);
     return hipGetLastError();
 }
+__device__ __forceinline__ uint32_t visit_rank(uint2 word, uint32_t node) { return word.y + __popc(word.x & ((1u << (node & 31)) - 1u)); }
 
 #define ZH_SCAN_CAP 256
 template <int D, int KIND>
 __global__ __launch_bounds__(256) void scan_sweep_kernel(const float *__restrict__ X, const float *__restrict__ Q,
                                                           const float *__restrict__ QQ, const uint2 *__restrict__ rowLeaf,
-                                                          uint32_t T, uint32_t RW, const uint32_t *__restrict__ visitBits,
-                                                          const uint4 *__restrict__ nodeVisit,
+                                                          uint32_t T, uint32_t RW, const uint2 *__restrict__ visitWords,
+                                                          const uint4 *__restrict__ visitRec,
                                                           const ZhGroup *__restrict__ groups, uint32_t GRP, uint64_t row_begin,
                                                           uint64_t row_end, int metric, int param,
                                                           uint64_t *__restrict__ keys, const uint32_t *__restrict__ run_if) {
@@ -1610,8 +1644,9 @@
             const unsigned long long rlw = __builtin_nontemporal_load(reinterpret_cast<const unsigned long long *>(ent + e));
             const uint2 rl = make_uint2((uint32_t)rlw, (uint32_t)(rlw >> 32));
             eWithin[j] = rl.y;
-            if (rl.x != 0xFFFFFFFFu && ((visitBits[rl.x >> 5] >> (rl.x & 31)) & 1u)) {
-                const uint4 nv = nodeVisit[rl.x];
+            const uint2 vw = rl.x != 0xFFFFFFFFu ? visitWords[rl.x >> 5] : make_uint2(0u, 0u);
+            if ((vw.x >> (rl.x & 31)) & 1u) {
+                const uint4 nv = visitRec[visit_rank(vw, rl.x)];
                 eC[j] = nv.x & 0x0FFFFFFFu; eGb[j] = nv.y; eB0[j] = nv.z;
                 eK0[j] = ((uint64_t)(nv.x >> 28) << 32) | nv.w;
             }
@@ -1758,8 +1793,8 @@
 template <int KIND>
 __global__ __launch_bounds__(256) void scan128_sweep_kernel(const float *__restrict__ X, const float *__restrict__ Q,
                                                              const float *__restrict__ QQ, const uint2 *__restrict__ rowLeaf,
-                                                             uint32_t T, uint32_t RW, const uint32_t *__restrict__ visitBits,
-                                                             const uint4 *__restrict__ nodeVisit,
+                                                             uint32_t T, uint32_t RW, const uint2 *__restrict__ visitWords,
+                                                             const uint4 *__restrict__ visitRec,
                                                              const ZhGroup *__restrict__ groups, uint32_t GRP, uint64_t row_begin,
                                                              uint64_t row_end, int metric, int param,
                                                              uint64_t *__restrict__ keys, const uint32_t *__restrict__ run_if) {
@@ -1789,8 +1824,9 @@
             const unsigned long long rlw = __builtin_nontemporal_load(reinterpret_cast<const unsigned long long *>(ent + e));
             const uint2 rl = make_uint2((uint32_t)rlw, (uint32_t)(rlw >> 32));
             eWithin[j] = rl.y;
-            if (rl.x != 0xFFFFFFFFu && ((visitBits[rl.x >> 5] >> (rl.x & 31)) & 1u)) {
-                const uint4 nv = nodeVisit[rl.x];
+            const uint2 vw = rl.x != 0xFFFFFFFFu ? visitWords[rl.x >> 5] : make_uint2(0u, 0u);
+            if ((vw.x >> (rl.x & 31)) & 1u) {
+                const uint4 nv = visitRec[visit_rank(vw, rl.x)];
                 eC[j] = nv.x & 0x0FFFFFFFu; eGb[j] = nv.y; eB0[j] = nv.z;
                 eK0[j] = ((uint64_t)(nv.x >> 28) << 32) | nv.w;
             }
@@ -1943,7 +1979,7 @@
 
 template <int D, int KIND>
 static hipError_t launch_scan_dk(const float *dX, uint64_t n_rows, const float *dQ, const float *dQQ, const uint2 *dRowLeaf,
-                                 uint32_t T, const uint32_t *dVisitBits, const uint4 *dNodeVisit, const ZhGroup *dGroups,
+                                 uint32_t T, const uint2 *dVisitWords, const uint4 *dVisitRec, const ZhGroup *dGroups,
                                  uint32_t group, int metric, int param, uint64_t *dKeys, const uint32_t *dRunIf, hipStream_t s) {
     const uint32_t RW = zh_scan_rows_per_wave(T);
     uint64_t rows_per_launch = zh_sweep_rows_per_launch(D);
@@ -1954,19 +1990,19 @@
         if (blocks > 0x7FFFFFFFull) return hipErrorInvalidValue;
         if constexpr (D == 128 && (KIND == K_L2 || KIND == K_COS))
             hipLaunchKernelGGL((scan128_sweep_kernel<KIND>), dim3((uint32_t)blocks), dim3(256), 0, s, dX, dQ, dQQ, dRowLeaf, T, RW,
-                               dVisitBits, dNodeVisit, dGroups, group, r, r_end, metric, param, dKeys, dRunIf);
+                               dVisitWords, dVisitRec, dGroups, group, r, r_end, metric, param, dKeys, dRunIf);
         else
             hipLaunchKernelGGL((scan_sweep_kernel<D, KIND>), dim3((uint32_t)blocks), dim3(256), 0, s, dX, dQ, dQQ, dRowLeaf, T, RW,
-                               dVisitBits, dNodeVisit, dGroups, group, r, r_end, metric, param, dKeys, dRunIf);
+                               dVisitWords, dVisitRec, dGroups, group, r, r_end, metric, param, dKeys, dRunIf);
     }
     return hipGetLastError();
 }
 template <int KIND>
 static hipError_t launch_scan_k(const float *dX, uint32_t d, uint64_t n_rows, const float *dQ, const float *dQQ,
-                                const uint2 *dRowLeaf, uint32_t T, const uint32_t *dVisitBits, const uint4 *dNodeVisit,
+                                const uint2 *dRowLeaf, uint32_t T, const uint2 *dVisitWords, const uint4 *dVisitRec,
                                 const ZhGroup *dGroups, uint32_t group, int metric, int param, uint64_t *dKeys, const uint32_t *dRunIf, hipStream_t s) {
 #define ZH_SCAN_CASE(DD) \
-    case DD: return launch_scan_dk<DD, KIND>(dX, n_rows, dQ, dQQ, dRowLeaf, T, dVisitBits, dNodeVisit, dGroups, group, metric, param, dKeys, dRunIf, s)
+    case DD: return launch_scan_dk<DD, KIND>(dX, n_rows, dQ, dQQ, dRowLeaf, T, dVisitWords, dVisitRec, dGroups, group, metric, param, dKeys, dRunIf, s)
     if constexpr (KIND == K_L2 || KIND == K_COS) {
         switch (d) {
             ZH_SCAN_CASE(64); ZH_SCAN_CASE(256); ZH_SCAN_CASE(512); ZH_SCAN_CASE(1024); ZH_SCAN_CASE(1536);
@@ -1980,12 +2016,12 @@
 #undef ZH_SCAN_CASE
 }
 hipError_t zh_launch_scan_sweep(const float *dX, uint32_t d, uint64_t n_rows, const float *dQ, const float *dQQ,
-                                const uint2 *dRowLeaf, uint32_t T, const uint32_t *dVisitBits, const uint4 *dNodeVisit,
+                                const uint2 *dRowLeaf, uint32_t T, const uint2 *dVisitWords, const uint4 *dVisitRec,
                                 const ZhGroup *dGroups, uint32_t group, int metric, int param, uint64_t *dKeys, const uint32_t *dRunIf,
                                 hipStream_t s) {
     if (!n_rows) return hipSuccess;
 #define ZH_KIND_CASE(K) \
-    case K: return launch_scan_k<K>(dX, d, n_rows, dQ, dQQ, dRowLeaf, T, dVisitBits, dNodeVisit, dGroups, group, metric, param, dKeys, dRunIf, s)
+    case K: return launch_scan_k<K>(dX, d, n_rows, dQ, dQQ, dRowLeaf, T, dVisitWords, dVisitRec, dGroups, group, metric, param, dKeys, dRunIf, s)
     switch (zh_kind_of(metric)) {
         ZH_KIND_CASE(K_COS);
         ZH_KIND_CASE(K_MAX);
@@ -1996,7 +2032,7 @@
         ZH_KIND_CASE(K_P4);
         ZH_KIND_CASE(K_HAMM);
         ZH_KIND_CASE(K_PP);
-    default: return launch_scan_k<K_L2>(dX, d, n_rows, dQ, dQQ, dRowLeaf, T, dVisitBits, dNodeVisit, dGroups, group, metric, param, dKeys, dRunIf, s);
+    default: return launch_scan_k<K_L2>(dX, d, n_rows, dQ, dQQ, dRowLeaf, T, dVisitWords, dVisitRec, dGroups, group, metric, param, dKeys, dRunIf, s);
     }
 #undef ZH_KIND_CASE
 }
```

After: 202,000. Within noise of the previous version (-0.6%).
